# zkonduit/ezkl

Measured on AMD Instinct MI355X. Metric: BN254 G1 MSM pts/s (2^20 points per GPU; NTT 2^22 elems/s in extra), higher is better.
Workload: dtype u32x8 (254-bit modular integer, Montgomery); 1 GPU; configs[1]: standalone 2^20-point BN254 G1 MSM (uniform scalars, try-and-increment bases) + 2^22 scalar-field NTT per GPU; parallelism=points sharded across 1 rank(s); all_gather of 64-B partials + host fold

## Files before the change

### ezkl_amd/backend.py

```python
import ctypes as C
import numpy as np
from . import lib as _l

_vp = C.c_void_p


def _p(a):
    return a.ctypes.data_as(_vp)


def _fe(a, shape_last=4):
    a = np.ascontiguousarray(a, dtype=np.uint64)
    if a.shape[-1] != shape_last:
        raise ValueError("expected trailing dimension %d" % shape_last)
    return a


def init(device=-1):
    _l.check(_l.load().ezkl_hip_init(C.c_int(device)), "ezkl_hip_init")


def synchronize():
    _l.check(_l.load().ezkl_hip_synchronize(), "ezkl_hip_synchronize")

# ... 293 lines not shown
    num_poly = message.shape[0] // n + 1
    polys = np.zeros((num_poly, n_rows, 4), np.uint64)
    polys[:, n:, :] = _to_mont(1)
    for i in range(message.shape[0]):
        polys[i // n, i % n] = message[i]
    out = np.zeros((num_poly, 8), np.uint64)
    arr = (C.c_void_p * num_poly)(*[polys[j].ctypes.data for j in range(num_poly)])
    _l.check(_l.load().ezkl_hip_msm_g1_batch(params._gl.h, arr, C.c_size_t(num_poly), C.c_size_t(n_rows), _p(out)),
             "ezkl_hip_msm_g1_batch")
    return out


def msm_g2(points, scalars):
    points, scalars = _fe(points, 16), _fe(scalars)
    if points.shape[0] != scalars.shape[0]:
        raise ValueError("one scalar per point")
    out = np.zeros(16, np.uint64)
    _l.check(_l.load().ezkl_hip_msm_g2(_p(points), _p(scalars), C.c_size_t(points.shape[0]), _p(out)), "ezkl_hip_msm_g2")
    return out


def g1_add_affine(a, b):
    a, b = _fe(a, 8), _fe(b, 8)
    out = np.zeros(8, np.uint64)
    _l.check(_l.load().ezkl_hip_g1_add_affine(_p(a), _p(b), _p(out)), "ezkl_hip_g1_add_affine")
    return out


def ntt(a, log_n, omega, inverse=False):
    a = _fe(a).copy()
    w = _fe(omega)
    _l.check(_l.load().ezkl_hip_ntt(_p(a), C.c_uint32(log_n), _p(w), C.c_int(1 if inverse else 0)), "ezkl_hip_ntt")
    return a


def ntt_dev(ptr, log_n, omega, inverse=False, batch=1, stride=None, stream=None):
    w = _fe(omega)
    stride = (1 << log_n) if stride is None else stride
    _l.check(_l.load().ezkl_hip_ntt_dev(_vp(ptr), C.c_uint32(log_n), _p(w), C.c_int(1 if inverse else 0),
                                         C.c_size_t(batch), C.c_size_t(stride), _stream_ptr(stream)), "ezkl_hip_ntt_dev")


def set_async(on):
    prev = C.c_int(0)
    _l.check(_l.load().ezkl_hip_set_async(C.c_int(1 if on else 0), C.byref(prev)), "ezkl_hip_set_async")
    return bool(prev.value)


def vec_op(op, a_ptr, b_ptr, out_ptr, n, stream=None):
    code = {"add": 0, "sub": 1, "mul": 2}[op]
    _l.check(_l.load().ezkl_hip_vec_op_dev(C.c_int(code), _vp(a_ptr), _vp(b_ptr), _vp(out_ptr), C.c_size_t(n),
                                            _stream_ptr(stream)), "ezkl_hip_vec_op_dev")


def permutation_sigma_dev(next_ptr, omega_col_ptr, delta_pows_ptr, n_columns, log_n, out_ptr, stream=None):
    _l.check(_l.load().ezkl_hip_permutation_sigma_dev(_vp(next_ptr), _vp(omega_col_ptr), _vp(delta_pows_ptr), C.c_uint32(n_columns), C.c_uint32(log_n),
                                                      _vp(out_ptr), _stream_ptr(stream)), "ezkl_hip_permutation_sigma_dev")


def vec_scale(a_ptr, scalar, out_ptr, n, stream=None):
    _l.check(_l.load().ezkl_hip_vec_scale_dev(_vp(a_ptr), _p(_fe(scalar)), _vp(out_ptr), C.c_size_t(n), _stream_ptr(stream)), "ezkl_hip_vec_scale_dev")


def vec_fill(out_ptr, value, n, stream=None):
    _l.check(_l.load().ezkl_hip_vec_fill_dev(_vp(out_ptr), _p(_fe(value)), C.c_size_t(n), _stream_ptr(stream)), "ezkl_hip_vec_fill_dev")


def coset_ntt_dev(in_ptr, out_ptr, k, ext_k, inverse=False, in_len=None, batch=1, stream=None):
    nin = (1 << ext_k) if inverse else (1 << k)
    _l.check(_l.load().ezkl_hip_coset_ntt_dev(_vp(in_ptr), _vp(out_ptr), C.c_size_t(batch), C.c_size_t(nin), C.c_size_t(1 << ext_k),
                                               C.c_uint32(k), C.c_uint32(ext_k), C.c_int(1 if inverse else 0), _stream_ptr(stream)),
             "ezkl_hip_coset_ntt_dev")


def coeff_to_cosets_dev(in_ptr, out_ptr, k, ext_k, batch=1, stream=None):
    _l.check(_l.load().ezkl_hip_coeff_to_cosets_dev(_vp(in_ptr), _vp(out_ptr), C.c_size_t(batch), C.c_size_t(1 << k), C.c_size_t(1 << ext_k),
                                                     C.c_uint32(k), C.c_uint32(ext_k), _stream_ptr(stream)), "ezkl_hip_coeff_to_cosets_dev")


def coeff_to_cosets_range_dev(in_ptr, out_ptr, k, ext_k, first_coset, n_cosets, batch=1, stream=None):
    _l.check(_l.load().ezkl_hip_coeff_to_cosets_range_dev(_vp(in_ptr), _vp(out_ptr), C.c_size_t(batch), C.c_size_t(1 << k), C.c_size_t(n_cosets << k),
                                                           C.c_uint32(k), C.c_uint32(ext_k), C.c_uint32(first_coset), C.c_uint32(n_cosets), _stream_ptr(stream)),
             "ezkl_hip_coeff_to_cosets_range_dev")


def cosets_transpose_dev(in_ptr, out_ptr, k, ext_k, to_natural=True, stream=None):
    _l.check(_l.load().ezkl_hip_cosets_transpose_dev(_vp(in_ptr), _vp(out_ptr), C.c_uint32(k), C.c_uint32(ext_k), C.c_int(1 if to_natural else 0),
                                                      _stream_ptr(stream)), "ezkl_hip_cosets_transpose_dev")


def divide_by_vanishing_dev(ptr, k, ext_k, stream=None):
    _l.check(_l.load().ezkl_hip_divide_by_vanishing_dev(_vp(ptr), C.c_uint32(k), C.c_uint32(ext_k), _stream_ptr(stream)),
             "ezkl_hip_divide_by_vanishing_dev")


def memcpy_h2d(dst_ptr, arr):
    arr = np.ascontiguousarray(arr)
    _l.check(_l.load().ezkl_hip_memcpy_h2d(_vp(dst_ptr), _p(arr), C.c_size_t(arr.nbytes)), "h2d")


def memcpy_d2h(src_ptr, nbytes):
    out = np.empty(nbytes, np.uint8)
    _l.check(_l.load().ezkl_hip_memcpy_d2h(_p(out), _vp(src_ptr), C.c_size_t(nbytes)), "d2h")
    return out


def prefix_scan(op, in_ptr, out_ptr, n, exclusive=False, stream=None):
    code = {"add": 0, "mul": 2}[op]
    _l.check(_l.load().ezkl_hip_prefix_scan_dev(C.c_int(code), C.c_int(1 if exclusive else 0), _vp(in_ptr), _vp(out_ptr),
                                                 C.c_size_t(n), _stream_ptr(stream)), "ezkl_hip_prefix_scan_dev")


def lookup_multiplicity(input_ptrs, table_ptr, n_rows, usable_rows, stream=None):
    out = DeviceBuffer(n_rows * 32)
    miss = C.c_uint32(0)
    arr = (C.c_void_p * max(1, len(input_ptrs)))(*input_ptrs)
    _l.check(_l.load().ezkl_hip_lookup_multiplicity_dev(arr, C.c_uint32(len(input_ptrs)), _vp(table_ptr), C.c_uint32(n_rows),
                                                         C.c_uint32(usable_rows), _vp(out.ptr), C.byref(miss), _stream_ptr(stream)),
             "ezkl_hip_lookup_multiplicity_dev")
    return out, int(miss.value)


def lookup_multiplicity_batch(inputs_per_lookup, table_ptrs, n_rows, usable_rows, stream=None):
    L = len(table_ptrs)
    outs = [DeviceBuffer(n_rows * 32) for _ in range(L)]
    flat = [p for ins in inputs_per_lookup for p in ins]
    which = [l for l, ins in enumerate(inputs_per_lookup) for _ in ins]
    miss = DeviceBuffer.from_numpy(np.zeros(1, np.uint32))
    a_in = (C.c_void_p * max(1, len(flat)))(*flat)
    a_which = (C.c_uint32 * max(1, len(which)))(*which)
    a_tab = (C.c_void_p * L)(*table_ptrs)
    a_out = (C.c_void_p * L)(*[o.ptr for o in outs])
    _l.check(_l.load().ezkl_hip_lookup_multiplicity_batch_dev(a_in, a_which, C.c_uint32(len(flat)), a_tab, C.c_uint32(L), C.c_uint32(n_rows), C.c_uint32(usable_rows),
                                                               a_out, _vp(miss.ptr), _stream_ptr(stream)), "ezkl_hip_lookup_multiplicity_batch_dev")
    return outs, int(miss.to_numpy(np.uint32, (1,))[0])


def _records(rec, counters, cap):
    cnt = counters.to_numpy(np.uint64)
    m = int(min(cnt[0], cap))
    r = rec.to_numpy(np.uint32)[:4 * m].reshape(m, 4) if m else np.zeros((0, 4), np.uint32)
    return [tuple(int(x) for x in row) for row in r], [int(x) for x in cnt]


def lookup_missing_rows(inputs_per_lookup, table_ptrs, n_rows, usable_rows, cap=1024, stream=None):
    L = len(table_ptrs)
    flat = [p for ins in inputs_per_lookup for p in ins]
    which = [l for l, ins in enumerate(inputs_per_lookup) for _ in ins]
    rec, cnt = DeviceBuffer(max(1, cap) * 16), DeviceBuffer.from_numpy(np.zeros(1 + L, np.uint64))
    a_in = (C.c_void_p * max(1, len(flat)))(*flat)
    a_which = (C.c_uint32 * max(1, len(which)))(*which)
    a_tab = (C.c_void_p * L)(*table_ptrs)
    _l.check(_l.load().ezkl_hip_lookup_missing_rows_dev(a_in, a_which, C.c_uint32(len(flat)), a_tab, C.c_uint32(L), C.c_uint32(n_rows), C.c_uint32(usable_rows),
                                                         _vp(rec.ptr), C.c_uint32(cap), _vp(cnt.ptr), _stream_ptr(stream)), "ezkl_hip_lookup_missing_rows_dev")
    return _records(rec, cnt, cap)


def copy_check(col_ptrs, next_ptr, log_n, cap=1024, stream=None):
    rec, cnt = DeviceBuffer(max(1, cap) * 16), DeviceBuffer.from_numpy(np.zeros(1, np.uint64))
    a = (C.c_void_p * max(1, len(col_ptrs)))(*col_ptrs)
    _l.check(_l.load().ezkl_hip_copy_check_dev(a, C.c_uint32(len(col_ptrs)), _vp(next_ptr), C.c_uint32(log_n), _vp(rec.ptr), C.c_uint32(cap), _vp(cnt.ptr),
                                                _stream_ptr(stream)), "ezkl_hip_copy_check_dev")
    return _records(rec, cnt, cap)


def eval_polynomial(coeffs_ptr, n, x, stream=None):
# ... 516 lines not shown
```

### ezkl_amd/csrc/capi.hip

```cpp
#include "common.hpp"
#include <string.h>
#include <atomic>
#include <algorithm>
#include <iterator>

namespace ezkl {

static std::mutex g_init_mu;
static constexpr int MAX_CTX = 64;
static std::atomic<Ctx*> g_ctxs[MAX_CTX];
static int g_ctx_device[MAX_CTX];
static std::atomic<int> g_n_ctx{0};
static thread_local int t_ctx = 0;
static std::atomic<int> g_last_hip_err{0};

int set_hip_error(hipError_t e, const char* what, const char* file, int line) {
    g_last_hip_err.store((int)e);
    fprintf(stderr, "[ezkl_hip] HIP error %d (%s) at %s:%d in %s\n", (int)e, hipGetErrorString(e), file, line, what);
    (void)hipGetLastError();
    return e == hipErrorOutOfMemory ? EZKL_ERR_NOMEM : EZKL_ERR_HIP;
}

static int device_count_checked(int* n) {
    *n = 0;
// ... 768 lines not shown
    for (size_t i = 0; i < count; i++)
        if (!scalars_dev[i]) return EZKL_ERR_INVALID;
    EZ_CTX(c);
    return msm_batch_push_many(c, reinterpret_cast<MsmBatch*>(batch), (const fe_t* const*)scalars_dev, count, c->stream);
}
int ezkl_hip_msm_batch_finish(ezkl_msm_batch_t batch, void* out, size_t capacity) {
    if (!batch || (!out && capacity)) return EZKL_ERR_INVALID;
    EZ_CTX(c);
    return msm_batch_finish(c, reinterpret_cast<MsmBatch*>(batch), out, capacity);
}
int ezkl_hip_g1_add_affine(const void* a, const void* b, void* out) {
    if (!a || !b || !out) return EZKL_ERR_INVALID;
    g1_add_affine_host(a, b, out);
    return EZKL_OK;
}

int ezkl_hip_ntt_dev(void* data, uint32_t log_n, const void* omega, int inverse, size_t batch, size_t stride, void* stream) {
    if (!data || !omega || batch == 0) return EZKL_ERR_INVALID;
    EZ_CTX(c);
    fe_t w;
    memcpy(&w, omega, 32);
    hipStream_t st = pick_stream(c, stream);
    int rc = ntt_run(c, st, (const fe_t*)data, (fe_t*)data, log_n, w, inverse != 0, batch, stride, stride, log_n, 0);
    if (rc) return rc;
    return finish(c, st, stream);
}
int ezkl_hip_ntt(void* data, uint32_t log_n, const void* omega, int inverse) {
    if (!data || !omega || log_n > 28) return EZKL_ERR_INVALID;
    EZ_CTX(c);
    size_t bytes = (size_t)32 << log_n;
    fe_t* d = nullptr;
    EZ_HIP(hipMalloc(&d, bytes));
    int rc = EZKL_OK;
    hipError_t e = hipMemcpyAsync(d, data, bytes, hipMemcpyHostToDevice, c->stream);
    if (e != hipSuccess) rc = set_hip_error(e, "h2d", __FILE__, __LINE__);
    if (!rc) rc = ezkl_hip_ntt_dev(d, log_n, omega, inverse, 1, (size_t)1 << log_n, nullptr);
    if (!rc) {
        e = copy_sync(c, data, d, bytes, hipMemcpyDeviceToHost);
        if (e != hipSuccess) rc = set_hip_error(e, "d2h", __FILE__, __LINE__);
    }
    (void)hipFree(d);
    return rc;
}

static fe_t domain_omega(uint32_t k, bool inverse) {
    fe_t w = fr_const(FrConst::ROOT);
    for (uint32_t i = k; i < 28; i++) w = Fr::sqr(w);
    return inverse ? Fr::inv(w) : w;
}

int ezkl_hip_coset_ntt_dev(const void* in, void* out, size_t batch, size_t in_stride, size_t out_stride,
                           uint32_t log_n, uint32_t log_n_ext, int inverse, void* stream) {
    if (!in || !out || batch == 0 || log_n > log_n_ext || log_n_ext > 28) return EZKL_ERR_INVALID;
    EZ_CTX(c);
    hipStream_t st = pick_stream(c, stream);
    fe_t w = domain_omega(log_n_ext, inverse != 0);
    int rc;
    if (!inverse)
        rc = ntt_run(c, st, (const fe_t*)in, (fe_t*)out, log_n_ext, w, false, batch, in_stride, out_stride, log_n, 1);
    else
        rc = ntt_run(c, st, (const fe_t*)in, (fe_t*)out, log_n_ext, w, true, batch, in_stride, out_stride, log_n_ext, 2);
    if (rc) return rc;
    return finish(c, st, stream);
}
int ezkl_hip_coeff_to_cosets_dev(const void* in, void* out, size_t batch, size_t in_stride, size_t out_stride, uint32_t log_n, uint32_t log_n_ext, void* stream) {
    if (!in || !out || in == out || batch == 0 || log_n > log_n_ext || log_n_ext > 28 || log_n_ext - log_n > 6) return EZKL_ERR_INVALID;
    EZ_CTX(c);
    hipStream_t st = pick_stream(c, stream);
    int rc = coset_cm_run(c, st, (const fe_t*)in, (fe_t*)out, log_n, log_n_ext, domain_omega(log_n, false), domain_omega(log_n_ext, false), batch, in_stride, out_stride);
    if (rc) return rc;
    return finish(c, st, stream);
}
int ezkl_hip_coeff_to_cosets_range_dev(const void* in, void* out, size_t batch, size_t in_stride, size_t out_stride, uint32_t log_n, uint32_t log_n_ext,
                                       uint32_t first_coset, uint32_t n_cosets, void* stream) {
    if (!in || !out || in == out || batch == 0 || log_n > log_n_ext || log_n_ext > 28 || log_n_ext - log_n > 6) return EZKL_ERR_INVALID;
    if (n_cosets == 0 || (n_cosets & (n_cosets - 1)) || (uint64_t)first_coset + n_cosets > (1ull << (log_n_ext - log_n))) return EZKL_ERR_INVALID;
    EZ_CTX(c);
    hipStream_t st = pick_stream(c, stream);
    int rc = coset_cm_run(c, st, (const fe_t*)in, (fe_t*)out, log_n, log_n_ext, domain_omega(log_n, false), domain_omega(log_n_ext, false), batch, in_stride, out_stride,
                          first_coset, n_cosets);
    if (rc) return rc;
    return finish(c, st, stream);
}
int ezkl_hip_cosets_transpose_dev(const void* in, void* out, uint32_t log_n, uint32_t log_n_ext, int to_natural, void* stream) {
    if (!in || !out || in == out || log_n > log_n_ext || log_n_ext > 28) return EZKL_ERR_INVALID;
    EZ_CTX(c);
    hipStream_t st = pick_stream(c, stream);
    int rc = cm_transpose(c, st, (const fe_t*)in, (fe_t*)out, log_n, log_n_ext - log_n, to_natural != 0);
    if (rc) return rc;
    return finish(c, st, stream);
}
int ezkl_hip_coset_ntt_batch(const void* const* in, void* const* out, size_t batch, uint32_t log_n, uint32_t log_n_ext, int inverse) {
    if (!in || !out || log_n > log_n_ext || log_n_ext > 28) return EZKL_ERR_INVALID;
    EZ_CTX(c);
    const size_t ne = (size_t)1 << log_n_ext, nin = inverse ? ne : ((size_t)1 << log_n);
    fe_t *din = nullptr, *dout = nullptr;
    EZ_HIP(hipMalloc(&din, nin * 32));
    EZ_HIP(hipMalloc(&dout, ne * 32));
    int rc = EZKL_OK;
    for (size_t b = 0; b < batch && !rc; b++) {
        hipError_t e = hipMemcpyAsync(din, in[b], nin * 32, hipMemcpyHostToDevice, c->stream);
        if (e != hipSuccess) { rc = set_hip_error(e, "h2d", __FILE__, __LINE__); break; }
        rc = ezkl_hip_coset_ntt_dev(din, dout, 1, nin, ne, log_n, log_n_ext, inverse, nullptr);
        if (rc) break;
        e = copy_sync(c, out[b], dout, ne * 32, hipMemcpyDeviceToHost);
        if (e != hipSuccess) rc = set_hip_error(e, "d2h", __FILE__, __LINE__);
    }
    (void)hipFree(din);
    (void)hipFree(dout);
    return rc;
}

int ezkl_hip_vec_op_dev(int op, const void* a, const void* b, void* o, size_t n, void* stream) {
    if (!a || !b || !o || op < 0 || op > 2) return EZKL_ERR_INVALID;
    EZ_CTX(c);
    hipStream_t st = pick_stream(c, stream);
    int rc = vec_op(c, st, op, (const fe_t*)a, (const fe_t*)b, (fe_t*)o, n);
    return rc ? rc : finish(c, st, stream);
}
int ezkl_hip_vec_fill_dev(void* o, const void* v, size_t n, void* stream) {
    if (!o || !v) return EZKL_ERR_INVALID;
    EZ_CTX(c);
    fe_t val;
    memcpy(&val, v, 32);
    hipStream_t st = pick_stream(c, stream);
    int rc = vec_fill(c, st, (fe_t*)o, val, n);
    return rc ? rc : finish(c, st, stream);
}
int ezkl_hip_permutation_sigma_dev(const void* next_dev, const void* omega_col_dev, const void* delta_pows_dev, uint32_t n_columns, uint32_t log_n,
                                   void* out_dev, void* stream) {
    if (!next_dev || !omega_col_dev || !delta_pows_dev || !out_dev || n_columns == 0 || log_n > 28) return EZKL_ERR_INVALID;
    if (((uint64_t)n_columns << log_n) > ((uint64_t)1 << 32)) return EZKL_ERR_INVALID;
    EZ_CTX(c);
    hipStream_t st = pick_stream(c, stream);
    int rc = perm_sigma(c, st, (const uint32_t*)next_dev, (const fe_t*)omega_col_dev, (const fe_t*)delta_pows_dev, log_n, n_columns, (fe_t*)out_dev);
    return rc ? rc : finish(c, st, stream);
}
int ezkl_hip_vec_scale_dev(const void* a, const void* s, void* o, size_t n, void* stream) {
    if (!a || !s || !o) return EZKL_ERR_INVALID;
    EZ_CTX(c);
    fe_t sc;
    memcpy(&sc, s, 32);
    hipStream_t st = pick_stream(c, stream);
    int rc = vec_scale(c, st, (const fe_t*)a, sc, (fe_t*)o, n);
    return rc ? rc : finish(c, st, stream);
}
int ezkl_hip_divide_by_vanishing_dev(void* a, uint32_t k, uint32_t ext_k, void* stream) {
    if (!a || k > ext_k || ext_k > 28) return EZKL_ERR_INVALID;
    EZ_CTX(c);
    return divide_by_vanishing(c, pick_stream(c, stream), (fe_t*)a, k, ext_k);
}
int ezkl_hip_batch_invert_dev(void* a, size_t n, void* stream) {
    if (!a) return EZKL_ERR_INVALID;
    EZ_CTX(c);
    hipStream_t st = pick_stream(c, stream);
    int rc = batch_invert(c, st, (fe_t*)a, n);
    return rc ? rc : finish(c, st, stream);
}

int ezkl_hip_lookup_multiplicity_dev(const void* const* inputs_dev, uint32_t n_inputs, const void* table_dev, uint32_t n_rows,
                                     uint32_t usable_rows, void* m_out_dev, uint32_t* out_missing, void* stream) {
    if (!table_dev || !m_out_dev || (n_inputs && !inputs_dev)) return EZKL_ERR_INVALID;
    for (uint32_t j = 0; j < n_inputs; j++)
        if (!inputs_dev[j]) return EZKL_ERR_INVALID;
    EZ_CTX(c);
    return lookup_multiplicity(c, pick_stream(c, stream), (const fe_t* const*)inputs_dev, n_inputs, (const fe_t*)table_dev, n_rows,
// ... 178 lines not shown
```

### ezkl_amd/csrc/common.hpp

```cpp
#pragma once
#include <hip/hip_runtime.h>
#include <stdint.h>
#include <stdio.h>
#include <map>
#include <mutex>
#include <string>
#include <vector>
#include <rocprofiler-sdk-roctx/roctx.h>
#include "../../include/ezkl_hip.h"
#include "field.hpp"

namespace ezkl {

struct Ctx {
    int device = -1;
    hipStream_t stream = nullptr;
    hipEvent_t order_event = nullptr;
    int num_cus = 256;
    std::recursive_mutex mu;
    struct EvRing {
        static constexpr unsigned N = 64;
        hipEvent_t e0[N], e1[N];
        bool made[N];
        uint64_t head = 0, tail = 0;
        double sum_ms = 0;
        uint64_t count = 0, skipped = 0;
        EvRing() { for (unsigned i = 0; i < N; i++) { e0[i] = e1[i] = nullptr; made[i] = false; } }
    };
    std::map<std::string, EvRing> events;
    struct Arena {
        void* ptr = nullptr;
        size_t bytes = 0;
        hipStream_t last_stream = nullptr;
        hipEvent_t last_event = nullptr;
        bool in_use = false;
    };
    Arena scratch, aux;
    std::map<hipStream_t, Arena> scratch_by_stream;
    void* msm_state = nullptr;
    void* ntt_state = nullptr;
    void* jit_state = nullptr;
    void* pool_state = nullptr;
    int index = 0;
    void* staging_state = nullptr;
    hipStream_t side_stream = nullptr;
};

Ctx* ctx();
int ctx_init(int device);
int ctx_count();
int ctx_bind(int idx);
int ctx_device_of(int idx);
int set_hip_error(hipError_t e, const char* what, const char* file, int line);
int arena_reserve(Ctx::Arena& a, size_t bytes, hipStream_t st, void** out);
int arena_done(Ctx::Arena& a, hipStream_t st);
int ev_pair(Ctx* c, const char* key, hipEvent_t* e0, hipEvent_t* e1);
int ev_harvest(Ctx::EvRing& r, bool all);
uint8_t* staging_acquire(Ctx* c, size_t bytes, void** token);
int staging_release(void* token, hipStream_t st);

#define EZ_HIP(call)                                                              \
    do {                                                                          \
        hipError_t _e = (call);                                                   \
        if (_e != hipSuccess) return ::ezkl::set_hip_error(_e, #call, __FILE__, __LINE__); \
    } while (0)

struct RoctxRange {
    explicit RoctxRange(const char* name) { roctxRangePushA(name); }
    ~RoctxRange() { roctxRangePop(); }
};

#define EZ_CTX(c)                                   \
    ::ezkl::RoctxRange _roctx(__func__);            \
    ::ezkl::Ctx* c = ::ezkl::ctx();                 \
    if (!c) return EZKL_ERR_NO_DEVICE;              \
    std::lock_guard<std::recursive_mutex> _lk(c->mu); \
    EZ_HIP(hipSetDevice(c->device))

static inline hipError_t stream_create_prio(hipStream_t* st, const char* env_name, int dflt) {
    int prio = dflt;
    if (const char* e = getenv(env_name)) prio = atoi(e);
    int lo = 0, hi = 0;
    if (hipDeviceGetStreamPriorityRange(&lo, &hi) != hipSuccess) { (void)hipGetLastError(); return hipStreamCreateWithFlags(st, hipStreamNonBlocking); }
    if (prio > lo) prio = lo;
    if (prio < hi) prio = hi;
    if (prio == 0) return hipStreamCreateWithFlags(st, hipStreamNonBlocking);
    return hipStreamCreateWithPriority(st, hipStreamNonBlocking, prio);
}
static inline Ctx::Arena& scratch_arena(Ctx* c, hipStream_t st) { return st == c->stream ? c->scratch : c->scratch_by_stream[st]; }
static inline hipStream_t pick_stream(Ctx* c, void* s) { return s ? (hipStream_t)s : c->stream; }
static inline unsigned cdiv(size_t a, size_t b) { return (unsigned)((a + b - 1) / b); }

struct Bases {
    fe_t* pts = nullptr;
    size_t n = 0;
};

int ntt_run(Ctx* c, hipStream_t st, const fe_t* in, fe_t* out, uint32_t log_n, const fe_t& omega, bool inverse_scale,
            size_t batch, size_t in_stride, size_t out_stride, uint32_t in_log_len, int coset_mode);
int coset_cm_run(Ctx* c, hipStream_t st, const fe_t* in, fe_t* out, uint32_t log_n, uint32_t log_ext, const fe_t& w_n, const fe_t& w_ext, size_t batch,
                 size_t in_stride, size_t out_stride, uint32_t first_coset = 0, uint32_t n_cosets = 0);
int cm_transpose(Ctx* c, hipStream_t st, const fe_t* in, fe_t* out, uint32_t log_n, uint32_t log_e, bool to_natural);
int msm_run(Ctx* c, hipStream_t st, const Bases* b, size_t base_offset, const fe_t* scalars_dev, size_t n,
            void* out_affine_host);
int msm_run_batch(Ctx* c, hipStream_t st, const Bases* b, size_t base_offset, const fe_t* const* scalars, size_t batch, size_t n,
                  void* out_host, bool small_scalars = false);
struct MsmUpload;
int msm_upload_begin(Ctx* c, const fe_t* const* host_cols, fe_t* const* dev_cols, size_t batch, size_t n, const fe_t* const* tails, size_t tail_start,
                     size_t tail_count, MsmUpload** out, const uint8_t* formats = nullptr);
int msm_upload_wait(MsmUpload* u, size_t j, hipStream_t st);
int msm_upload_commit(Ctx* c, MsmUpload* u, const Bases* b, size_t commit_first, size_t commit_count, void* out_host);
int msm_upload_end(MsmUpload* u);
struct MsmBatch;
int msm_batch_begin(Ctx* c, hipStream_t st, const Bases* b, size_t base_offset, size_t n, MsmBatch** out);
int msm_batch_push(Ctx* c, MsmBatch* mb, const fe_t* scalars_dev);
int msm_batch_push_many(Ctx* c, MsmBatch* mb, const fe_t* const* cols, size_t count, hipStream_t after);
int msm_batch_finish(Ctx* c, MsmBatch* mb, void* out_host, size_t capacity);
int vec_op(Ctx* c, hipStream_t st, int op, const fe_t* a, const fe_t* b, fe_t* o, size_t n);
int vec_fill(Ctx* c, hipStream_t st, fe_t* o, const fe_t& v, size_t n);
int vec_scale(Ctx* c, hipStream_t st, const fe_t* a, const fe_t& s, fe_t* o, size_t n);
int perm_sigma(Ctx* c, hipStream_t st, const uint32_t* next, const fe_t* omega_col, const fe_t* delta_pows, uint32_t log_n, uint32_t m, fe_t* out);
int divide_by_vanishing(Ctx* c, hipStream_t st, fe_t* a, uint32_t k, uint32_t ext_k);
int batch_invert(Ctx* c, hipStream_t st, fe_t* a, size_t n);
int lookup_multiplicity_batch(Ctx* c, hipStream_t st, const fe_t* const* inputs, const uint32_t* which, uint32_t n_items, const fe_t* const* tables,
                              uint32_t n_lookups, uint32_t n_rows, uint32_t usable, fe_t* const* m_outs, uint32_t* missing_host, uint32_t* missing_dev);
int lookup_multiplicity(Ctx* c, hipStream_t st, const fe_t* const* inputs, uint32_t n_inputs, const fe_t* table, uint32_t n_rows,
                        uint32_t usable, fe_t* m_out, uint32_t* missing_host, uint32_t* missing_dev);
int eval_poly(Ctx* c, hipStream_t st, const fe_t* coeffs, size_t n, const fe_t& x, void* out_host);
int prefix_scan(Ctx* c, hipStream_t st, int op, int exclusive, const fe_t* in, fe_t* out, size_t n);
int eval_poly_batch(Ctx* c, hipStream_t st, const fe_t* const* coeffs, const fe_t* xs, uint32_t m, size_t n, void* out_host);
int lincomb(Ctx* c, hipStream_t st, const fe_t* const* in, const fe_t* coeffs, uint32_t m, fe_t* out, size_t n, int accumulate);
int kate_division(Ctx* c, hipStream_t st, const fe_t* a, const fe_t& z, fe_t* out, size_t n);
int chacha20_fr(Ctx* c, hipStream_t st, const uint32_t key[8], uint64_t stream, size_t first, fe_t* out, size_t n);
bool msm_upload_is_open();
int msm_run_concurrent(Ctx* c, std::unique_lock<std::recursive_mutex>& lk, const Bases* b, size_t base_offset, const fe_t* scalars, size_t n, void* out_host);
int msm_call_start(Ctx* c, std::unique_lock<std::recursive_mutex>& lk, const Bases* b, size_t base_offset, const fe_t* scalars, size_t n, int* slot_out);
int msm_call_finish(Ctx* c, std::unique_lock<std::recursive_mutex>& lk, int slot, void* out_host);
int eval_program(Ctx* c, hipStream_t st, const ezkl_program_t* p, fe_t* out, bool ordered);
int eval_jit_compile_only(const ezkl_program_t* p);
int eval_jit_source_only(const ezkl_program_t* p, char* out, size_t cap, size_t* len);
int eval_check_source_only(const ezkl_program_t* p, const uint32_t* slots, uint32_t n_checks, char* out, size_t cap, size_t* len);
int eval_check(Ctx* c, hipStream_t st, const ezkl_program_t* p, const uint32_t* slots, uint32_t n_checks, uint32_t row_lo, uint32_t row_hi, void* rec,
               uint32_t cap, void* count);
int lookup_missing_rows(Ctx* c, hipStream_t st, const fe_t* const* inputs, const uint32_t* which, uint32_t n_items, const fe_t* const* tables,
                        uint32_t n_lookups, uint32_t n_rows, uint32_t usable, void* rec, uint32_t cap, void* count);
int copy_check(Ctx* c, hipStream_t st, const fe_t* const* cols, uint32_t m, const uint32_t* next, uint32_t log_n, void* rec, uint32_t cap, void* count);
int eval_prepare(Ctx* c, const ezkl_program_t* p);
int eval_schedule_only(const ezkl_program_t* p, uint32_t* out_code);
void eval_jit_stats(uint64_t* compiled, uint64_t* from_disk, uint64_t* hits);
int ubench(Ctx* c, const char* which, double* out);
void msm_table_drop(const Bases* b);
int msm_table_prepare(Ctx* c, const Bases* b);
int g1_mul_fixed(Ctx* c, hipStream_t st, const void* base_host, const fe_t* scalars, size_t n, void* out_dev);
int gen_bases(Ctx* c, hipStream_t st, uint64_t seed, size_t first, size_t n, void* out_dev);
int g1_to_lagrange(Ctx* c, hipStream_t st, const void* g_dev, uint32_t log_n, fe_t* tw_mont, const fe_t& ninv_mont, void* out_dev);
void g1_add_affine_host(const void* a, const void* b, void* out);
int g2_msm(Ctx* c, hipStream_t st, const void* pts_host, const void* scalars_host, size_t n, void* out_host);

}
```

### ezkl_amd/csrc/field29.hpp

```cpp
#pragma once
#include "field.hpp"
#include "montmul29_gen.hpp"

#ifndef EZKL_FQ29_ILP
#define EZKL_FQ29_ILP 0
#endif
#ifndef EZKL_FUSED_Y
#define EZKL_FUSED_Y 1
#endif
namespace ezkl {

struct f29_t {
    uint32_t v[9];
};
static constexpr uint32_t M29 = (1u << 29) - 1;

template <class CT, bool IS_FQ>
struct Field29 {
    typedef CT C;
    typedef uint32_t u32x9 __attribute__((ext_vector_type(9)));
    EZ_D static void mul_asm(const uint32_t (&a)[9], const uint32_t (&b)[9], uint32_t (&r)[9]) {
        if (IS_FQ) {
#if EZKL_FQ29_ILP
            mont_mul29i_fq(a, b, r);
#else
            mont_mul29_fq(a, b, r);
#endif
        } else mont_mul29_fr(a, b, r);
    }

    EZ_D static f29_t zero() {
        f29_t r;
#pragma unroll
        for (int i = 0; i < 9; i++) r.v[i] = 0;
        return r;
    }
    EZ_D static f29_t one() {
        f29_t r;
#pragma unroll
        for (int i = 0; i < 9; i++) r.v[i] = C::ONE[i];
        return r;
    }
    EZ_D static bool limbs_zero(const f29_t& a) {
        uint32_t o = 0;
#pragma unroll
        for (int i = 0; i < 9; i++) o |= a.v[i];
        return o == 0;
    }
    __device__ __attribute__((noinline)) static u32x9 mul_call(u32x9 a, u32x9 b) {
        uint32_t x[9], y[9], r[9];
#pragma unroll
        for (int i = 0; i < 9; i++) { x[i] = a[i]; y[i] = b[i]; }
        mul_asm(x, y, r);
        u32x9 o;
#pragma unroll
        for (int i = 0; i < 9; i++) o[i] = r[i];
        return o;
    }
    EZ_D static f29_t mul(const f29_t& a, const f29_t& b) {
        f29_t r;
        mul_asm(a.v, b.v, r.v);
        return r;
    }
    EZ_D static f29_t mul2add(const f29_t& a, const f29_t& b, const f29_t& c, const f29_t& d) {
        static_assert(IS_FQ, "generated for Fq only");
        f29_t r;
        mont_mul2add29_fq(a.v, b.v, c.v, d.v, r.v);
        return r;
    }
    EZ_D static f29_t mul_cold(const f29_t& a, const f29_t& b) {
        u32x9 x, y;
#pragma unroll
        for (int i = 0; i < 9; i++) { x[i] = a.v[i]; y[i] = b.v[i]; }
        u32x9 o = mul_call(x, y);
        f29_t r;
#pragma unroll
        for (int i = 0; i < 9; i++) r.v[i] = o[i];
        return r;
    }
    EZ_D static f29_t sqr(const f29_t& a) {
        f29_t r;
        if (IS_FQ) {
#if EZKL_FQ29_ILP
            mont_sqr29i_fq(a.v, r.v);
#else
            mont_sqr29_fq(a.v, r.v);
#endif
        } else mont_sqr29_fr(a.v, r.v);
        return r;
    }
    EZ_D static f29_t sqr_cold(const f29_t& a) { return mul_cold(a, a); }
    EZ_D static f29_t add(const f29_t& a, const f29_t& b) {
        f29_t r;
#pragma unroll
        for (int i = 0; i < 9; i++) r.v[i] = a.v[i] + b.v[i];
        return r;
    }
    template <int KI>
    EZ_D static f29_t sub(const f29_t& a, const f29_t& b) {
        f29_t r;
#pragma unroll
        for (int i = 0; i < 9; i++) r.v[i] = a.v[i] + (C::SUBC[KI][i] - b.v[i]);
        return r;
    }
    template <int KI>
    EZ_D static f29_t neg(const f29_t& b) {
        f29_t r;
#pragma unroll
        for (int i = 0; i < 9; i++) r.v[i] = C::SUBC[KI][i] - b.v[i];
        return r;
    }
    EZ_D static f29_t normalize(const f29_t& a) {
        f29_t r = a;
#pragma unroll
        for (int i = 0; i < 8; i++) {
            r.v[i + 1] += r.v[i] >> 29;
            r.v[i] &= M29;
        }
        return r;
    }
    EZ_D static bool is_zero_mod_p(const f29_t& a) {
        const uint32_t j = (a.v[0] * C::P0INV) & M29;
        if (j >= 32) return false;
        uint32_t carry = 0, diff = 0;
#pragma unroll
        for (int i = 0; i < 9; i++) {
            const uint64_t t = (uint64_t)j * C::P[i] + carry;
            const uint32_t limb = i < 8 ? ((uint32_t)t & M29) : (uint32_t)t;
            carry = i < 8 ? (uint32_t)(t >> 29) : 0;
            diff |= limb ^ a.v[i];
        }
        return diff == 0;
    }
    template <int KI>
    EZ_D static f29_t cond_sub(const f29_t& x) {
        f29_t t;
#pragma unroll
        for (int i = 0; i < 9; i++) t.v[i] = x.v[i] + C::CSUB[KI][i];
        t = normalize(t);
        const bool ge = (t.v[8] >> 29) != 0;
        t.v[8] &= M29;
        f29_t r;
#pragma unroll
        for (int i = 0; i < 9; i++) r.v[i] = ge ? t.v[i] : x.v[i];
        return r;
    }
    EZ_D static f29_t canonical(const f29_t& x) {
        constexpr uint32_t D = (uint32_t)(C::P[8] + 1u);
        constexpr uint64_t MAGIC = (((uint64_t)1 << 51) + D - 1) / D;
        const uint32_t q = (uint32_t)(((uint64_t)x.v[8] * MAGIC) >> 51);
        f29_t r;
        uint64_t acc = 0;
#pragma unroll
        for (int i = 0; i < 9; i++) {
            acc += (uint64_t)q * C::CSUB[0][i] + x.v[i];
            r.v[i] = (uint32_t)acc & M29;
            acc >>= 29;
        }
        return cond_sub<0>(r);
    }
    EZ_D static fe_t pack(const f29_t& a) {
        fe_t w;
#pragma unroll
        for (int j = 0; j < 8; j++) {
            const int bit = 32 * j, lo = bit / 29, sh = bit - 29 * lo;
            uint32_t acc = a.v[lo] >> sh;
            const int have = 29 - sh;
            if (lo + 1 < 9) acc |= a.v[lo + 1] << have;
            if (have + 29 < 32 && lo + 2 < 9) acc |= a.v[lo + 2] << (have + 29);
            w.v[j] = acc;
        }
        return w;
    }
    EZ_D static f29_t unpack(const fe_t& w) {
        f29_t r;
#pragma unroll
        for (int i = 0; i < 8; i++) {
            const int bit = 29 * i, word = bit >> 5, sh = bit & 31;
            const uint32_t lo = w.v[word], hi = word + 1 < 8 ? w.v[word + 1] : 0u;
            r.v[i] = (sh ? __builtin_amdgcn_alignbit(hi, lo, sh) : lo) & M29;
        }
        r.v[8] = w.v[7] >> 8;
        return r;
    }
};

typedef Field29<Fq29C, true> Fq29;
typedef Field29<Fr29C, false> Fr29;

EZ_D f29_t ld_f29(const f29_t* p) {
    f29_t r;
#pragma unroll
    for (int i = 0; i < 9; i++) r.v[i] = p->v[i];
    return r;
}
EZ_D void st_f29(f29_t* p, const f29_t& a) {
#pragma unroll
    for (int i = 0; i < 9; i++) p->v[i] = a.v[i];
}

}
```

### ezkl_amd/csrc/montmul29_gen.hpp

```cpp
#pragma once
#ifndef __HIPCC_RTC__
#include <stdint.h>
#endif
namespace ezkl {
struct Fq29C {
    static constexpr uint32_t P[9] = {0x187cfd47u, 0x010460b6u, 0x1c72a34fu, 0x02d522d0u, 0x1585d978u, 0x02db40c0u, 0x00a6e141u, 0x0e5c2634u, 0x0030644eu};
    static constexpr uint32_t ONE[9] = {0x157ccc21u, 0x141c2758u, 0x185230d3u, 0x014c0419u, 0x0aa36fb9u, 0x1d4240ceu, 0x11d54c07u, 0x052ac7a8u, 0x000dc836u};
    static constexpr uint32_t P0INV = 0x1b799c77u;
    static constexpr uint32_t SUBC[7][9] = {
        {0x30f9fa8eu, 0x2208c16cu, 0x38e5469du, 0x25aa45a0u, 0x2b0bb2efu, 0x25b68180u, 0x214dc281u, 0x3cb84c67u, 0x0060c89bu},
        {0x21f3f51cu, 0x241182dau, 0x31ca8d3bu, 0x2b548b42u, 0x361765dfu, 0x2b6d0301u, 0x229b8503u, 0x397098cfu, 0x00c19138u},
        {0x23e7ea38u, 0x282305b5u, 0x23951a77u, 0x36a91686u, 0x2c2ecbbfu, 0x36da0604u, 0x25370a07u, 0x32e1319fu, 0x01832272u},
        {0x27cfd470u, 0x30460b6bu, 0x272a34efu, 0x2d522d0du, 0x385d9780u, 0x2db40c09u, 0x2a6e1410u, 0x25c2633fu, 0x030644e6u},
        {0x2f9fa8e0u, 0x208c16d7u, 0x2e5469e0u, 0x3aa45a1bu, 0x30bb2f01u, 0x3b681814u, 0x34dc2821u, 0x2b84c67fu, 0x060c89cdu},
        {0x3f3f51c0u, 0x21182dafu, 0x3ca8d3c1u, 0x3548b437u, 0x21765e04u, 0x36d0302au, 0x29b85044u, 0x37098d00u, 0x0c19139bu},
        {0x3e7ea380u, 0x22305b60u, 0x3951a783u, 0x2a916870u, 0x22ecbc0au, 0x2da06055u, 0x3370a08au, 0x2e131a01u, 0x18322738u},
    };
    static constexpr uint32_t CSUB[4][9] = {
        {0x078302b9u, 0x1efb9f49u, 0x038d5cb0u, 0x1d2add2fu, 0x0a7a2687u, 0x1d24bf3fu, 0x1f591ebeu, 0x11a3d9cbu, 0x1fcf9bb1u},
        {0x0f060572u, 0x1df73e92u, 0x071ab961u, 0x1a55ba5eu, 0x14f44d0fu, 0x1a497e7eu, 0x1eb23d7du, 0x0347b397u, 0x1f9f3763u},
        {0x1e0c0ae4u, 0x1bee7d24u, 0x0e3572c3u, 0x14ab74bcu, 0x09e89a1fu, 0x1492fcfdu, 0x1d647afbu, 0x068f672fu, 0x1f3e6ec6u},
        {0x1c1815c8u, 0x17dcfa49u, 0x1c6ae587u, 0x0956e978u, 0x13d1343fu, 0x0925f9fau, 0x1ac8f5f7u, 0x0d1ece5fu, 0x1e7cdd8cu},
    };
    static constexpr uint32_t R261_32[8] = {0x157ccc21u, 0x4e8384ebu, 0x0ce148c3u, 0xfb90a602u, 0x819caa36u, 0x5301fa84u, 0x563d4475u, 0x0dc83629u};
};
struct Fr29C {
    static constexpr uint32_t P[9] = {0x10000001u, 0x1f0fac9fu, 0x0e5c2450u, 0x07d090f3u, 0x1585d283u, 0x02db40c0u, 0x00a6e141u, 0x0e5c2634u, 0x0030644eu};
    static constexpr uint32_t ONE[9] = {0x0fffff57u, 0x1ea70ab4u, 0x052c068bu, 0x17504f49u, 0x0aa8075bu, 0x1d4240ceu, 0x11d54c07u, 0x052ac7a8u, 0x000dc836u};
    static constexpr uint32_t P0INV = 0x10000001u;
    static constexpr uint32_t SUBC[7][9] = {
        {0x20000002u, 0x3e1f593eu, 0x3cb848a0u, 0x2fa121e5u, 0x2b0ba505u, 0x25b68180u, 0x214dc281u, 0x3cb84c67u, 0x0060c89bu},
        {0x20000004u, 0x3c3eb27du, 0x39709142u, 0x3f4243ccu, 0x36174a0bu, 0x2b6d0301u, 0x229b8503u, 0x397098cfu, 0x00c19138u},
        {0x20000008u, 0x387d64fbu, 0x32e12286u, 0x3e84879au, 0x2c2e9418u, 0x36da0604u, 0x25370a07u, 0x32e1319fu, 0x01832272u},
        {0x20000010u, 0x30fac9f7u, 0x25c2450eu, 0x3d090f36u, 0x385d2832u, 0x2db40c09u, 0x2a6e1410u, 0x25c2633fu, 0x030644e6u},
        {0x20000020u, 0x21f593efu, 0x2b848a1eu, 0x3a121e6du, 0x30ba5066u, 0x3b681814u, 0x34dc2821u, 0x2b84c67fu, 0x060c89cdu},
        {0x20000040u, 0x23eb27dfu, 0x3709143du, 0x34243cdbu, 0x2174a0ceu, 0x36d0302au, 0x29b85044u, 0x37098d00u, 0x0c19139bu},
        {0x20000080u, 0x27d64fbfu, 0x2e12287bu, 0x284879b8u, 0x22e9419eu, 0x2da06055u, 0x3370a08au, 0x2e131a01u, 0x18322738u},
    };
    static constexpr uint32_t CSUB[4][9] = {
        {0x0fffffffu, 0x00f05360u, 0x11a3dbafu, 0x182f6f0cu, 0x0a7a2d7cu, 0x1d24bf3fu, 0x1f591ebeu, 0x11a3d9cbu, 0x1fcf9bb1u},
        {0x1ffffffeu, 0x01e0a6c0u, 0x0347b75eu, 0x105ede19u, 0x14f45af9u, 0x1a497e7eu, 0x1eb23d7du, 0x0347b397u, 0x1f9f3763u},
        {0x1ffffffcu, 0x03c14d81u, 0x068f6ebcu, 0x00bdbc32u, 0x09e8b5f3u, 0x1492fcfdu, 0x1d647afbu, 0x068f672fu, 0x1f3e6ec6u},
        {0x1ffffff8u, 0x07829b03u, 0x0d1edd78u, 0x017b7864u, 0x13d16be6u, 0x0925f9fau, 0x1ac8f5f7u, 0x0d1ece5fu, 0x1e7cdd8cu},
    };
    static constexpr uint32_t R261_32[8] = {0x8fffff57u, 0x2fd4e156u, 0xa494b01au, 0x75bba827u, 0x819caa80u, 0x5301fa84u, 0x563d4475u, 0x0dc83629u};
};
__device__ __forceinline__ void mont_mul29_fq(const uint32_t (&a)[9], const uint32_t (&b)[9], uint32_t (&r)[9]) {
    asm("s_mov_b32 s16, 0x187cfd47\n\t"
        "s_mov_b32 s17, 0x010460b6\n\t"
        "s_mov_b32 s18, 0x1c72a34f\n\t"
        "s_mov_b32 s19, 0x02d522d0\n\t"
        "s_mov_b32 s20, 0x1585d978\n\t"
        "s_mov_b32 s21, 0x02db40c0\n\t"
        "s_mov_b32 s22, 0x00a6e141\n\t"
        "s_mov_b32 s23, 0x0e5c2634\n\t"
        "s_mov_b32 s24, 0x0030644e\n\t"
        "s_mov_b32 s25, 0x04866389\n\t"
        "s_mov_b32 s26, 0x1fffffff\n\t"
        "v_mad_u64_u32 v[16:17], vcc, %[a0], %[b0], 0\n\t"
        "v_mul_lo_u32 %[r0], v16, s25\n\t"
        "v_and_b32 %[r0], s26, %[r0]\n\t"
        "v_mad_u64_u32 v[16:17], vcc, %[r0], s16, v[16:17]\n\t"
        "v_lshrrev_b64 v[16:17], 29, v[16:17]\n\t"
        "v_mad_u64_u32 v[16:17], vcc, %[a0], %[b1], v[16:17]\n\t"
        "v_mad_u64_u32 v[16:17], vcc, %[a1], %[b0], v[16:17]\n\t"
        "v_mad_u64_u32 v[16:17], vcc, %[r0], s17, v[16:17]\n\t"
        "v_mul_lo_u32 %[r1], v16, s25\n\t"
        "v_and_b32 %[r1], s26, %[r1]\n\t"
        "v_mad_u64_u32 v[16:17], vcc, %[r1], s16, v[16:17]\n\t"
        "v_lshrrev_b64 v[16:17], 29, v[16:17]\n\t"
        "v_mad_u64_u32 v[16:17], vcc, %[a0], %[b2], v[16:17]\n\t"
        "v_mad_u64_u32 v[16:17], vcc, %[a1], %[b1], v[16:17]\n\t"
        "v_mad_u64_u32 v[16:17], vcc, %[a2], %[b0], v[16:17]\n\t"
        "v_mad_u64_u32 v[16:17], vcc, %[r0], s18, v[16:17]\n\t"
        "v_mad_u64_u32 v[16:17], vcc, %[r1], s17, v[16:17]\n\t"
        "v_mul_lo_u32 %[r2], v16, s25\n\t"
        "v_and_b32 %[r2], s26, %[r2]\n\t"
        "v_mad_u64_u32 v[16:17], vcc, %[r2], s16, v[16:17]\n\t"
        "v_lshrrev_b64 v[16:17], 29, v[16:17]\n\t"
        "v_mad_u64_u32 v[16:17], vcc, %[a0], %[b3], v[16:17]\n\t"
        "v_mad_u64_u32 v[16:17], vcc, %[a1], %[b2], v[16:17]\n\t"
        "v_mad_u64_u32 v[16:17], vcc, %[a2], %[b1], v[16:17]\n\t"
        "v_mad_u64_u32 v[16:17], vcc, %[a3], %[b0], v[16:17]\n\t"
        "v_mad_u64_u32 v[16:17], vcc, %[r0], s19, v[16:17]\n\t"
        "v_mad_u64_u32 v[16:17], vcc, %[r1], s18, v[16:17]\n\t"
        "v_mad_u64_u32 v[16:17], vcc, %[r2], s17, v[16:17]\n\t"
        "v_mul_lo_u32 %[r3], v16, s25\n\t"
        "v_and_b32 %[r3], s26, %[r3]\n\t"
        "v_mad_u64_u32 v[16:17], vcc, %[r3], s16, v[16:17]\n\t"
        "v_lshrrev_b64 v[16:17], 29, v[16:17]\n\t"
        "v_mad_u64_u32 v[16:17], vcc, %[a0], %[b4], v[16:17]\n\t"
        "v_mad_u64_u32 v[16:17], vcc, %[a1], %[b3], v[16:17]\n\t"
        "v_mad_u64_u32 v[16:17], vcc, %[a2], %[b2], v[16:17]\n\t"
        "v_mad_u64_u32 v[16:17], vcc, %[a3], %[b1], v[16:17]\n\t"
        "v_mad_u64_u32 v[16:17], vcc, %[a4], %[b0], v[16:17]\n\t"
        "v_mad_u64_u32 v[16:17], vcc, %[r0], s20, v[16:17]\n\t"
        "v_mad_u64_u32 v[16:17], vcc, %[r1], s19, v[16:17]\n\t"
        "v_mad_u64_u32 v[16:17], vcc, %[r2], s18, v[16:17]\n\t"
        "v_mad_u64_u32 v[16:17], vcc, %[r3], s17, v[16:17]\n\t"
        "v_mul_lo_u32 %[r4], v16, s25\n\t"
        "v_and_b32 %[r4], s26, %[r4]\n\t"
        "v_mad_u64_u32 v[16:17], vcc, %[r4], s16, v[16:17]\n\t"
        "v_lshrrev_b64 v[16:17], 29, v[16:17]\n\t"
        "v_mad_u64_u32 v[16:17], vcc, %[a0], %[b5], v[16:17]\n\t"
        "v_mad_u64_u32 v[16:17], vcc, %[a1], %[b4], v[16:17]\n\t"
        "v_mad_u64_u32 v[16:17], vcc, %[a2], %[b3], v[16:17]\n\t"
        "v_mad_u64_u32 v[16:17], vcc, %[a3], %[b2], v[16:17]\n\t"
        "v_mad_u64_u32 v[16:17], vcc, %[a4], %[b1], v[16:17]\n\t"
        "v_mad_u64_u32 v[16:17], vcc, %[a5], %[b0], v[16:17]\n\t"
        "v_mad_u64_u32 v[16:17], vcc, %[r0], s21, v[16:17]\n\t"
        "v_mad_u64_u32 v[16:17], vcc, %[r1], s20, v[16:17]\n\t"
        "v_mad_u64_u32 v[16:17], vcc, %[r2], s19, v[16:17]\n\t"
        "v_mad_u64_u32 v[16:17], vcc, %[r3], s18, v[16:17]\n\t"
        "v_mad_u64_u32 v[16:17], vcc, %[r4], s17, v[16:17]\n\t"
        "v_mul_lo_u32 %[r5], v16, s25\n\t"
        "v_and_b32 %[r5], s26, %[r5]\n\t"
        "v_mad_u64_u32 v[16:17], vcc, %[r5], s16, v[16:17]\n\t"
        "v_lshrrev_b64 v[16:17], 29, v[16:17]\n\t"
        "v_mad_u64_u32 v[16:17], vcc, %[a0], %[b6], v[16:17]\n\t"
        "v_mad_u64_u32 v[16:17], vcc, %[a1], %[b5], v[16:17]\n\t"
        "v_mad_u64_u32 v[16:17], vcc, %[a2], %[b4], v[16:17]\n\t"
        "v_mad_u64_u32 v[16:17], vcc, %[a3], %[b3], v[16:17]\n\t"
        "v_mad_u64_u32 v[16:17], vcc, %[a4], %[b2], v[16:17]\n\t"
        "v_mad_u64_u32 v[16:17], vcc, %[a5], %[b1], v[16:17]\n\t"
        "v_mad_u64_u32 v[16:17], vcc, %[a6], %[b0], v[16:17]\n\t"
        "v_mad_u64_u32 v[16:17], vcc, %[r0], s22, v[16:17]\n\t"
        "v_mad_u64_u32 v[16:17], vcc, %[r1], s21, v[16:17]\n\t"
        "v_mad_u64_u32 v[16:17], vcc, %[r2], s20, v[16:17]\n\t"
// ... 1665 lines not shown
        "v_mad_u64_u32 v[16:17], vcc, %[r5], s20, v[16:17]\n\t"
        "v_mad_u64_u32 v[18:19], vcc, %[a7], %[b3], v[18:19]\n\t"
        "v_mad_u64_u32 v[16:17], vcc, %[r6], s19, v[16:17]\n\t"
        "v_mad_u64_u32 v[18:19], vcc, %[a8], %[b2], v[18:19]\n\t"
        "v_mad_u64_u32 v[16:17], vcc, %[r7], s18, v[16:17]\n\t"
        "v_mad_u64_u32 v[16:17], vcc, %[r8], s17, v[16:17]\n\t"
        "v_and_b32 %[r0], s26, v16\n\t"
        "v_lshrrev_b64 v[16:17], 29, v[16:17]\n\t"
        "v_lshl_add_u64 v[16:17], v[18:19], 0, v[16:17]\n\t"
        "v_mad_u64_u32 v[18:19], vcc, %[a3], %[b8], 0\n\t"
        "v_mad_u64_u32 v[16:17], vcc, %[r2], s24, v[16:17]\n\t"
        "v_mad_u64_u32 v[18:19], vcc, %[a4], %[b7], v[18:19]\n\t"
        "v_mad_u64_u32 v[16:17], vcc, %[r3], s23, v[16:17]\n\t"
        "v_mad_u64_u32 v[18:19], vcc, %[a5], %[b6], v[18:19]\n\t"
        "v_mad_u64_u32 v[16:17], vcc, %[r4], s22, v[16:17]\n\t"
        "v_mad_u64_u32 v[18:19], vcc, %[a6], %[b5], v[18:19]\n\t"
        "v_mad_u64_u32 v[16:17], vcc, %[r5], s21, v[16:17]\n\t"
        "v_mad_u64_u32 v[18:19], vcc, %[a7], %[b4], v[18:19]\n\t"
        "v_mad_u64_u32 v[16:17], vcc, %[r6], s20, v[16:17]\n\t"
        "v_mad_u64_u32 v[18:19], vcc, %[a8], %[b3], v[18:19]\n\t"
        "v_mad_u64_u32 v[16:17], vcc, %[r7], s19, v[16:17]\n\t"
        "v_mad_u64_u32 v[16:17], vcc, %[r8], s18, v[16:17]\n\t"
        "v_and_b32 %[r1], s26, v16\n\t"
        "v_lshrrev_b64 v[16:17], 29, v[16:17]\n\t"
        "v_lshl_add_u64 v[16:17], v[18:19], 0, v[16:17]\n\t"
        "v_mad_u64_u32 v[18:19], vcc, %[a4], %[b8], 0\n\t"
        "v_mad_u64_u32 v[16:17], vcc, %[r3], s24, v[16:17]\n\t"
        "v_mad_u64_u32 v[18:19], vcc, %[a5], %[b7], v[18:19]\n\t"
        "v_mad_u64_u32 v[16:17], vcc, %[r4], s23, v[16:17]\n\t"
        "v_mad_u64_u32 v[18:19], vcc, %[a6], %[b6], v[18:19]\n\t"
        "v_mad_u64_u32 v[16:17], vcc, %[r5], s22, v[16:17]\n\t"
        "v_mad_u64_u32 v[18:19], vcc, %[a7], %[b5], v[18:19]\n\t"
        "v_mad_u64_u32 v[16:17], vcc, %[r6], s21, v[16:17]\n\t"
        "v_mad_u64_u32 v[18:19], vcc, %[a8], %[b4], v[18:19]\n\t"
        "v_mad_u64_u32 v[16:17], vcc, %[r7], s20, v[16:17]\n\t"
        "v_mad_u64_u32 v[16:17], vcc, %[r8], s19, v[16:17]\n\t"
        "v_and_b32 %[r2], s26, v16\n\t"
        "v_lshrrev_b64 v[16:17], 29, v[16:17]\n\t"
        "v_lshl_add_u64 v[16:17], v[18:19], 0, v[16:17]\n\t"
        "v_mad_u64_u32 v[18:19], vcc, %[a5], %[b8], 0\n\t"
        "v_mad_u64_u32 v[16:17], vcc, %[r4], s24, v[16:17]\n\t"
        "v_mad_u64_u32 v[18:19], vcc, %[a6], %[b7], v[18:19]\n\t"
        "v_mad_u64_u32 v[16:17], vcc, %[r5], s23, v[16:17]\n\t"
        "v_mad_u64_u32 v[18:19], vcc, %[a7], %[b6], v[18:19]\n\t"
        "v_mad_u64_u32 v[16:17], vcc, %[r6], s22, v[16:17]\n\t"
        "v_mad_u64_u32 v[18:19], vcc, %[a8], %[b5], v[18:19]\n\t"
        "v_mad_u64_u32 v[16:17], vcc, %[r7], s21, v[16:17]\n\t"
        "v_mad_u64_u32 v[16:17], vcc, %[r8], s20, v[16:17]\n\t"
        "v_and_b32 %[r3], s26, v16\n\t"
        "v_lshrrev_b64 v[16:17], 29, v[16:17]\n\t"
        "v_lshl_add_u64 v[16:17], v[18:19], 0, v[16:17]\n\t"
        "v_mad_u64_u32 v[18:19], vcc, %[a6], %[b8], 0\n\t"
        "v_mad_u64_u32 v[16:17], vcc, %[r5], s24, v[16:17]\n\t"
        "v_mad_u64_u32 v[18:19], vcc, %[a7], %[b7], v[18:19]\n\t"
        "v_mad_u64_u32 v[16:17], vcc, %[r6], s23, v[16:17]\n\t"
        "v_mad_u64_u32 v[18:19], vcc, %[a8], %[b6], v[18:19]\n\t"
        "v_mad_u64_u32 v[16:17], vcc, %[r7], s22, v[16:17]\n\t"
        "v_mad_u64_u32 v[16:17], vcc, %[r8], s21, v[16:17]\n\t"
        "v_and_b32 %[r4], s26, v16\n\t"
        "v_lshrrev_b64 v[16:17], 29, v[16:17]\n\t"
        "v_lshl_add_u64 v[16:17], v[18:19], 0, v[16:17]\n\t"
        "v_mad_u64_u32 v[18:19], vcc, %[a7], %[b8], 0\n\t"
        "v_mad_u64_u32 v[16:17], vcc, %[r6], s24, v[16:17]\n\t"
        "v_mad_u64_u32 v[18:19], vcc, %[a8], %[b7], v[18:19]\n\t"
        "v_mad_u64_u32 v[16:17], vcc, %[r7], s23, v[16:17]\n\t"
        "v_mad_u64_u32 v[16:17], vcc, %[r8], s22, v[16:17]\n\t"
        "v_and_b32 %[r5], s26, v16\n\t"
        "v_lshrrev_b64 v[16:17], 29, v[16:17]\n\t"
        "v_lshl_add_u64 v[16:17], v[18:19], 0, v[16:17]\n\t"
        "v_mad_u64_u32 v[18:19], vcc, %[a8], %[b8], 0\n\t"
        "v_mad_u64_u32 v[16:17], vcc, %[r7], s24, v[16:17]\n\t"
        "v_mad_u64_u32 v[16:17], vcc, %[r8], s23, v[16:17]\n\t"
        "v_and_b32 %[r6], s26, v16\n\t"
        "v_lshrrev_b64 v[16:17], 29, v[16:17]\n\t"
        "v_lshl_add_u64 v[16:17], v[18:19], 0, v[16:17]\n\t"
        "v_mad_u64_u32 v[16:17], vcc, %[r8], s24, v[16:17]\n\t"
        "v_and_b32 %[r7], s26, v16\n\t"
        "v_lshrrev_b64 v[16:17], 29, v[16:17]\n\t"
        "v_mov_b32 %[r8], v16\n\t"
        : [r0] "=&v"(r[0]), [r1] "=&v"(r[1]), [r2] "=&v"(r[2]), [r3] "=&v"(r[3]), [r4] "=&v"(r[4]), [r5] "=&v"(r[5]), [r6] "=&v"(r[6]), [r7] "=&v"(r[7]), [r8] "=&v"(r[8])
        : [a0] "v"(a[0]), [a1] "v"(a[1]), [a2] "v"(a[2]), [a3] "v"(a[3]), [a4] "v"(a[4]), [a5] "v"(a[5]), [a6] "v"(a[6]), [a7] "v"(a[7]), [a8] "v"(a[8]), [b0] "v"(b[0]), [b1] "v"(b[1]), [b2] "v"(b[2]), [b3] "v"(b[3]), [b4] "v"(b[4]), [b5] "v"(b[5]), [b6] "v"(b[6]), [b7] "v"(b[7]), [b8] "v"(b[8])
        : "v16", "v17", "v18", "v19", "s16", "s17", "s18", "s19", "s20", "s21", "s22", "s23", "s24", "s25", "s26", "vcc");
}
}
```

### ezkl_amd/csrc/ntt.hip

```cpp
#include "common.hpp"
#include "field29.hpp"
#include <string.h>


namespace ezkl {

static constexpr uint32_t NTT_LOG_TILE = 10;
static constexpr uint32_t NTT_LOG_SINGLE = 11;

struct PassArgs {
    const fe_t* in;
    fe_t* out;
    size_t in_stride, out_stride;
    const fe_t* tw_inter;
    uint32_t log_n, log_r, log_m, log_tile;
    uint32_t last, first;
    uint32_t in_log_len;
    uint32_t coset_pre;
    uint32_t post;
    uint32_t npass, log_radix[4];
    uint32_t k1_major;
    fe_t zeta[2];
    fe_t post_c[3];
    uint32_t cm, cm_log_e, cm_first, cm_log_cnt;
    const f29_t* tw_stage29;
    const f29_t* tw_pre29;
    uint32_t lds_stages;
};

EZ_D void lds_put29(uint2* d, uint32_t* d8, uint32_t tile, uint32_t e, const f29_t& x) {
#pragma unroll
    for (int q = 0; q < 4; q++) d[q * tile + e] = make_uint2(x.v[2 * q], x.v[2 * q + 1]);
    d8[e] = x.v[8];
}
EZ_D f29_t lds_get29(const uint2* d, const uint32_t* d8, uint32_t tile, uint32_t e) {
    f29_t x;
#pragma unroll
    for (int q = 0; q < 4; q++) {
        uint2 t = d[q * tile + e];
        x.v[2 * q] = t.x;
        x.v[2 * q + 1] = t.y;
    }
    x.v[8] = d8[e];
    return x;
}
template <int G, int NTT_THREADS, bool FROM_TABLE>
__device__ __forceinline__ void ntt_superstage29(uint2* data, uint32_t* d8, const f29_t* tw, uint32_t TILE, uint32_t logC, bool unit1, uint32_t s, uint32_t tid) {
    constexpr uint32_t M = 1u << G;
    const uint32_t C = 1u << logC;
    const uint32_t lh = s - 1, h = 1u << lh;
    const uint32_t ngroups = TILE >> G;
    for (uint32_t gid = tid; gid < ngroups; gid += NTT_THREADS) {
        const uint32_t c = gid & (C - 1), q = gid >> logC;
        const uint32_t o = q & (h - 1), blk = q >> lh;
        const uint32_t r0 = (blk << (lh + G)) + o;
        f29_t x[M];
#pragma unroll
        for (uint32_t i = 0; i < M; i++) x[i] = lds_get29(data, d8, TILE, ((r0 + i * h) << logC) + c);
#pragma unroll
        for (int t = 0; t < G; t++) {
            const uint32_t half = 1u << t, st = s + t;
            const uint32_t base = (1u << (st - 1)) - 1u;
#pragma unroll
            for (uint32_t i = 0; i < M; i++) {
                if (i & half) continue;
                if (unit1 && st == 1) {
                    const f29_t v = x[i + half];
                    x[i + half] = Fr29::sub<2>(x[i], v);
                    x[i] = Fr29::add(x[i], v);
                } else if (unit1 && st == 2 && (i & 1u) == 0) {
                    const f29_t v = Fr29::normalize(x[i + half]);
                    x[i + half] = Fr29::sub<4>(x[i], v);
                    x[i] = Fr29::add(x[i], v);
                } else {
                    const uint32_t off = o + (i & (half - 1)) * h;
                    const f29_t w = ld_f29(tw + base + off);
                    const f29_t v = Fr29::mul(x[i + half], w);
                    x[i + half] = Fr29::sub<1>(x[i], v);
                    x[i] = Fr29::add(x[i], v);
                }
            }
        }
#pragma unroll
        for (uint32_t i = 0; i < M; i++) lds_put29(data, d8, TILE, ((r0 + i * h) << logC) + c, Fr29::normalize(x[i]));
    }
}

template <int NTT_THREADS>
__global__ __launch_bounds__(NTT_THREADS) void ntt_pass_kernel(PassArgs a) {
    extern __shared__ __attribute__((aligned(16))) unsigned char smem[];
    const uint32_t TILE = 1u << a.log_tile;
    const uint32_t logC = a.log_tile - a.log_r, C = 1u << logC;
    const uint32_t log_s = a.log_m - a.log_r, S = 1u << log_s;
    uint2* data = reinterpret_cast<uint2*>(smem);
    uint32_t* d8 = reinterpret_cast<uint32_t*>(smem + 32u * TILE);
    f29_t* tloc = reinterpret_cast<f29_t*>(smem + 36u * TILE);
    const uint32_t tid = threadIdx.x, tile = blockIdx.x;
    const uint32_t cm_l = a.cm ? (blockIdx.y & ((1u << a.cm_log_cnt) - 1u)) : 0u, cm_col = a.cm ? (blockIdx.y >> a.cm_log_cnt) : blockIdx.y;
    const uint32_t cm_b = a.cm_first + cm_l;
    const bool twisted = a.cm && a.first;
    const fe_t* in = a.in + (size_t)(twisted ? cm_col : blockIdx.y) * a.in_stride;
    fe_t* out = (a.cm && a.last) ? a.out + (size_t)cm_col * a.out_stride + ((size_t)cm_l << a.log_n) : a.out + (size_t)blockIdx.y * a.out_stride;
    const fe_t* tw_inter = a.tw_inter ? a.tw_inter + (twisted ? ((size_t)cm_b << a.log_n) : 0) : nullptr;
    const f29_t* tws = twisted ? a.tw_pre29 + ((size_t)cm_b << a.log_r) : a.tw_stage29;
    for (uint32_t j = tid; j + 1 < (1u << a.lds_stages); j += NTT_THREADS) st_f29(tloc + j, ld_f29(tws + j));

    uint32_t n_blocks = 1u << (a.log_n - a.log_r);
    uint32_t sblk = a.npass >= 2 ? (n_blocks >> a.log_radix[0]) : 1u;
    auto col_base = [&](uint32_t c) -> size_t {
        if (!a.last) {
            uint32_t colid = tile * C + c;
            return ((size_t)(colid >> log_s) << a.log_m) + (colid & (S - 1));
        }
        uint32_t blk;
        if (a.k1_major) {
            uint32_t rest = tile % sblk, k10 = (tile / sblk) * C;
            blk = (k10 + c) * sblk + rest;
        } else {
            blk = tile * C + c;
        }
        return (size_t)blk << a.log_r;
    };

    const size_t in_len = (size_t)1 << a.in_log_len;
    auto load_one = [&](uint32_t e, size_t& addr_out) -> fe_t {
        uint32_t c = e & (C - 1), i1 = e >> logC;
        size_t addr = col_base(c) + ((size_t)i1 << log_s);
        addr_out = addr;
        if (!a.first || addr < in_len) return ld_fe(in + addr);
        return Fr::zero();
    };
    auto put_one = [&](uint32_t e, size_t addr, const fe_t& raw) {
        f29_t x = Fr29::unpack(raw);
        if (a.first && a.coset_pre && addr < in_len) {
            uint32_t m3 = (uint32_t)(addr % 3);
            if (m3) x = Fr29::mul(x, Fr29::unpack(a.zeta[m3 - 1]));
        }
        e = (a.log_r ? ((__brev(e >> logC) >> (32 - a.log_r)) << logC) : 0u) | (e & (C - 1));
        lds_put29(data, d8, TILE, e, x);
    };
    if (TILE == 4 * NTT_THREADS) {
        fe_t x[4];
        size_t ad[4];
#pragma unroll
        for (int i = 0; i < 4; i++) x[i] = load_one(tid + i * NTT_THREADS, ad[i]);
#pragma unroll
        for (int i = 0; i < 4; i++) put_one(tid + i * NTT_THREADS, ad[i], x[i]);
    } else {
        for (uint32_t e = tid; e < TILE; e += NTT_THREADS) {
            size_t ad;
            fe_t x = load_one(e, ad);
            put_one(e, ad, x);
        }
    }
    __syncthreads();

    for (uint32_t s = 1; s <= a.log_r;) {
        const uint32_t g = a.log_r - s >= 1 ? 2u : 1u;
        if (s > a.lds_stages) {
            if (g == 2) ntt_superstage29<2, NTT_THREADS, true>(data, d8, tws, TILE, logC, !twisted, s, tid);
            else ntt_superstage29<1, NTT_THREADS, true>(data, d8, tws, TILE, logC, !twisted, s, tid);
        } else {
            if (g == 2) ntt_superstage29<2, NTT_THREADS, false>(data, d8, tloc, TILE, logC, !twisted, s, tid);
            else ntt_superstage29<1, NTT_THREADS, false>(data, d8, tloc, TILE, logC, !twisted, s, tid);
        }
        __syncthreads();
        s += g;
    }

    auto store_one = [&](uint32_t e, const fe_t* twp) {
        uint32_t c = e & (C - 1), k1 = e >> logC;
        f29_t x = lds_get29(data, d8, TILE, (k1 << logC) + c);
        if (!a.last) {
            uint32_t colid = tile * C + c;
            uint32_t pos = (k1 << log_s) + (colid & (S - 1));
            x = Fr29::mul(x, Fr29::unpack(twp ? *twp : ld_fe(tw_inter + pos)));
            st_fe(out + (((size_t)(colid >> log_s) << a.log_m) + pos), Fr29::pack(x));
        } else {
            uint32_t blk = (uint32_t)(col_base(c) >> a.log_r);
            size_t oidx = 0;
            uint32_t rem = blk, lw = a.log_n - a.log_r, shift = 0;
            for (uint32_t p = 0; p + 1 < a.npass; p++) {
                lw -= a.log_radix[p];
                uint32_t kp = rem >> lw;
                rem &= (1u << lw) - 1;
                oidx += (size_t)kp << shift;
                shift += a.log_radix[p];
            }
            oidx += (size_t)k1 << shift;
            x = a.post ? Fr29::cond_sub<0>(Fr29::mul(x, Fr29::unpack(a.post_c[oidx % 3]))) : Fr29::canonical(x);
            st_fe(out + oidx, Fr29::pack(x));
        }
    };
    if (TILE == 4 * NTT_THREADS && !a.last) {
        fe_t tw[4];
#pragma unroll
        for (int i = 0; i < 4; i++) {
            uint32_t e = tid + i * NTT_THREADS, c = e & (C - 1), k1 = e >> logC;
            tw[i] = ld_fe(tw_inter + ((k1 << log_s) + ((tile * C + c) & (S - 1))));
        }
#pragma unroll
        for (int i = 0; i < 4; i++) store_one(tid + i * NTT_THREADS, &tw[i]);
    } else {
        for (uint32_t e = tid; e < TILE; e += NTT_THREADS) store_one(e, nullptr);
    }
}

__global__ void ntt_twiddle_kernel(fe_t* out, uint32_t count, uint64_t mult, uint32_t log_n, uint32_t log_s,
                                   int mode, const fe_t* pow2tab, fe_t init) {
    uint32_t idx = blockIdx.x * blockDim.x + threadIdx.x;
    if (idx >= count) return;
    uint64_t e;
    if (mode == 0) e = (uint64_t)idx * mult;
    else e = (uint64_t)(idx & ((1u << log_s) - 1)) * (uint64_t)(idx >> log_s) * mult;
    e &= ((uint64_t)1 << log_n) - 1;
    fe_t acc = init;
    for (uint32_t b = 0; b < log_n; b++)
        if ((e >> b) & 1) acc = Fr::mul(acc, ld_fe(pow2tab + b));
    st_fe(out + idx, acc);
}


__global__ void ntt_coset_table_kernel(fe_t* out, f29_t* out29, uint32_t cnt, uint32_t log_e, uint32_t log_ext, uint32_t log_s, int mode, const fe_t* pow2tab,
                                       fe_t z0, fe_t z1, fe_t z2) {
    const size_t idx = (size_t)blockIdx.x * blockDim.x + threadIdx.x;
    if (idx >= ((size_t)cnt << log_e)) return;
    const uint64_t b = idx / cnt, m = idx % cnt;
    uint64_t e, z;
    if (mode == 0) {
        uint32_t st = 1;
        while (((uint64_t)1 << st) - 1 <= m) st++;
        const uint64_t o = m - (((uint64_t)1 << (st - 1)) - 1), log_nn = log_ext - log_e;
        if (st > log_nn) {
            if (out29) st_f29(out29 + idx, Fr29::zero());
            else st_fe(out + idx, Fr::zero());
            return;
        }
        const uint64_t q = (uint64_t)1 << (log_nn - st);
        e = q * (b + (o << log_e));
        z = q % 3;
    } else {
        const uint64_t i2 = m & (((uint64_t)1 << log_s) - 1), k1 = m >> log_s;
        e = ((i2 * k1) << log_e) + b * i2;
        z = i2 % 3;
    }
    e &= ((uint64_t)1 << log_ext) - 1;
    fe_t acc = z == 0 ? z0 : (z == 1 ? z1 : z2);
    for (uint32_t q = 0; q < log_ext; q++)
        if ((e >> q) & 1) acc = Fr::mul(acc, ld_fe(pow2tab + q));
    if (out29) st_f29(out29 + idx, Fr29::unpack(acc));
    else st_fe(out + idx, acc);
}
__global__ __launch_bounds__(256) void ntt_cm_transpose_kernel(const fe_t* in, fe_t* out, uint32_t log_n, uint32_t log_e, int to_natural) {
    const size_t j = (size_t)blockIdx.x * blockDim.x + threadIdx.x;
    if (j >> log_n) return;
    const uint32_t E = 1u << log_e;
    for (uint32_t b = 0; b < E; b++) {
        const size_t cm = ((size_t)b << log_n) + j, nat = (j << log_e) + b;
        if (to_natural) st_fe(out + nat, ld_fe(in + cm));
        else st_fe(out + cm, ld_fe(in + nat));
    }
}

struct NttPlan {
    uint32_t log_n = 0;
    int npass = 0;
    uint32_t log_radix[4] = {0, 0, 0, 0};
    fe_t* tw_inter[4] = {nullptr, nullptr, nullptr, nullptr};
    f29_t* stage29 = nullptr;
    fe_t n_inv;
};

struct CosetTables {
    f29_t* pre29 = nullptr;
    fe_t* inter = nullptr;
};
struct NttState {
    std::map<std::string, NttPlan*> plans;
    std::map<uint64_t, CosetTables> coset_tables;
    bool attrs_set = false;
};
static NttState& ntt_state() {
    Ctx* c = ctx();
    if (!c->ntt_state) c->ntt_state = new NttState();
    return *static_cast<NttState*>(c->ntt_state);
}
#define g_plans (ntt_state().plans)
#define g_coset_tables (ntt_state().coset_tables)

static uint32_t ntt_lds_stages(uint32_t log_r) { return log_r < 6 ? log_r : 6; }
static size_t ntt_lds_bytes(uint32_t log_tile, uint32_t log_r) { return 36u * ((size_t)1 << log_tile) + 36u * ((size_t)1 << ntt_lds_stages(log_r)); }
static fe_t ntt_domain_one() { return Fr::from_u64(32); }

static uint32_t ntt_max_radix() {
    static const uint32_t v = [] {
        const char* e = getenv("EZKL_NTT_MAXR");
        const int x = e ? atoi(e) : 0;
        return (uint32_t)(x >= 6 && x <= 11 ? x : 8);
    }();
    return v;
}
static void plan_radices(uint32_t log_n, NttPlan* p) {
    if (log_n <= NTT_LOG_SINGLE) {
        p->npass = 1;
        p->log_radix[0] = log_n;
        return;
    }
    const uint32_t maxr = ntt_max_radix();
    int np = (int)((log_n + maxr - 1) / maxr);
    if (np < 2) np = 2;
    if (np > 4) np = 4;
    p->npass = np;
    uint32_t base = log_n / np, extra = log_n % np;
    for (int i = 0; i < np; i++) p->log_radix[i] = base + ((uint32_t)i < extra ? 1 : 0);
}
static uint32_t pass_log_tile(uint32_t log_r) { return log_r >= 11 ? log_r : (log_r + 2 > NTT_LOG_TILE ? log_r + 2 : NTT_LOG_TILE); }
static void launch_pass(const PassArgs& a, uint32_t tiles, unsigned blocks_y, size_t lds, hipStream_t st) {
    if (a.npass > 1 && a.log_tile == 12) hipLaunchKernelGGL(ntt_pass_kernel<1024>, dim3(tiles, blocks_y), dim3(1024), lds, st, a);
    else if (a.npass > 1 && a.log_tile == 11) hipLaunchKernelGGL(ntt_pass_kernel<512>, dim3(tiles, blocks_y), dim3(512), lds, st, a);
    else hipLaunchKernelGGL(ntt_pass_kernel<256>, dim3(tiles, blocks_y), dim3(256), lds, st, a);
}
static int ntt_kernel_attrs() {
    bool& attr_set = ntt_state().attrs_set;
    if (!attr_set) {
        EZ_HIP(hipFuncSetAttribute((const void*)ntt_pass_kernel<256>, hipFuncAttributeMaxDynamicSharedMemorySize, 160 * 1024));
        EZ_HIP(hipFuncSetAttribute((const void*)ntt_pass_kernel<512>, hipFuncAttributeMaxDynamicSharedMemorySize, 160 * 1024));
        EZ_HIP(hipFuncSetAttribute((const void*)ntt_pass_kernel<1024>, hipFuncAttributeMaxDynamicSharedMemorySize, 160 * 1024));
        attr_set = true;
    }
    return EZKL_OK;
}

static int plan_get(Ctx* c, hipStream_t st, uint32_t log_n, const fe_t& omega, NttPlan** out) {
    std::string key((const char*)&omega, sizeof(fe_t));
    key.push_back((char)log_n);
    auto it = g_plans.find(key);
    if (it != g_plans.end()) { *out = it->second; return EZKL_OK; }
    NttPlan* p = new NttPlan();
    p->log_n = log_n;
    plan_radices(log_n, p);
    std::vector<fe_t> pow2(log_n ? log_n : 1);
    fe_t w = omega;
    for (uint32_t b = 0; b < log_n; b++) { pow2[b] = w; w = Fr::sqr(w); }
    p->n_inv = Fr::inv(Fr::from_u64((uint64_t)1 << log_n));
    fe_t* d_pow2 = nullptr;
    EZ_HIP(hipMalloc(&d_pow2, sizeof(fe_t) * pow2.size()));
    EZ_HIP(hipMemcpyAsync(d_pow2, pow2.data(), sizeof(fe_t) * pow2.size(), hipMemcpyHostToDevice, st));
    uint32_t log_m = log_n;
    const fe_t one = ntt_domain_one();
    {
        uint32_t maxlr = 0;
        for (int i = 0; i < p->npass; i++) maxlr = p->log_radix[i] > maxlr ? p->log_radix[i] : maxlr;
        const uint32_t cnt = 1u << maxlr;
        EZ_HIP(hipMalloc(&p->stage29, sizeof(f29_t) * cnt));
        hipLaunchKernelGGL(ntt_coset_table_kernel, dim3(cdiv(cnt, 256)), dim3(256), 0, st, (fe_t*)nullptr, p->stage29, cnt, 0u, log_n, 0u, 0, d_pow2, one, one, one);
    }
    for (int i = 0; i < p->npass; i++) {
        uint32_t lr = p->log_radix[i];
        if (i + 1 < p->npass) {
            uint32_t cnt = 1u << log_m;
            EZ_HIP(hipMalloc(&p->tw_inter[i], sizeof(fe_t) * (size_t)cnt));
            hipLaunchKernelGGL(ntt_twiddle_kernel, dim3(cdiv(cnt, 256)), dim3(256), 0, st, p->tw_inter[i], cnt,
                               (uint64_t)1 << (log_n - log_m), log_n, log_m - lr, 1, d_pow2, one);
        }
        log_m -= lr;
    }
    EZ_HIP(hipGetLastError());
    EZ_HIP(hipStreamSynchronize(st));
    EZ_HIP(hipFree(d_pow2));
    g_plans[key] = p;
    *out = p;
    return EZKL_OK;
}

static int ntt_run_chunk(Ctx* c, hipStream_t st, const fe_t* in, fe_t* out, uint32_t log_n, const fe_t& omega, bool inverse_scale,
                         size_t batch, size_t in_stride, size_t out_stride, uint32_t in_log_len, int coset_mode);

int ntt_run(Ctx* c, hipStream_t st, const fe_t* in, fe_t* out, uint32_t log_n, const fe_t& omega, bool inverse_scale,
            size_t batch, size_t in_stride, size_t out_stride, uint32_t in_log_len, int coset_mode) {
    if (log_n > 28 || in_log_len > log_n || batch == 0) return EZKL_ERR_INVALID;
    size_t group = ((size_t)4 << 30) / ((size_t)32 << log_n);
    if (group < 1) group = 1;
    if (group > 32768) group = 32768;
    for (size_t b0 = 0; b0 < batch; b0 += group) {
        size_t nb = batch - b0 < group ? batch - b0 : group;
        int rc = ntt_run_chunk(c, st, in + b0 * in_stride, out + b0 * out_stride, log_n, omega, inverse_scale, nb, in_stride, out_stride,
                               in_log_len, coset_mode);
        if (rc) return rc;
    }
    return EZKL_OK;
}

static int ntt_run_chunk(Ctx* c, hipStream_t st, const fe_t* in, fe_t* out, uint32_t log_n, const fe_t& omega, bool inverse_scale,
                         size_t batch, size_t in_stride, size_t out_stride, uint32_t in_log_len, int coset_mode) {
    NttPlan* p = nullptr;
    int rc = plan_get(c, st, log_n, omega, &p);
    if (rc) return rc;
    const size_t n = (size_t)1 << log_n;
    if ((rc = ntt_kernel_attrs())) return rc;
    fe_t* work = nullptr;
    if (p->npass > 1) {
        rc = arena_reserve(scratch_arena(c, st), batch * n * sizeof(fe_t), st, (void**)&work);
        if (rc) return rc;
    }
    const fe_t dom = ntt_domain_one();
    const fe_t zeta = Fr::mul(fr_const(FrConst::ZETA), dom), zeta2 = Fr::mul(fr_const(FrConst::ZETA2), dom);
    uint32_t log_m = log_n;
    hipEvent_t e0 = nullptr, e1 = nullptr;
    const char* tmode = getenv("EZKL_HIP_TIMING");
    const bool timed = !(tmode && !strcmp(tmode, "none"));
    if (timed) {
        rc = ev_pair(c, coset_mode ? "coset_ntt" : "ntt", &e0, &e1);
        if (rc) return rc;
        EZ_HIP(hipEventRecord(e0, st));
    }
    for (int i = 0; i < p->npass; i++) {
        PassArgs a;
        memset(&a, 0, sizeof a);
        const bool first = (i == 0), last = (i + 1 == p->npass);
        a.in = first ? in : work;
        a.in_stride = first ? in_stride : n;
        a.out = last ? out : work;
        a.out_stride = last ? out_stride : n;
        a.tw_inter = p->tw_inter[i];
        a.tw_stage29 = p->stage29;
        a.log_n = log_n;
        a.log_r = p->log_radix[i];
        a.lds_stages = ntt_lds_stages(a.log_r);
        a.log_m = log_m;
        a.log_tile = p->npass == 1 ? log_n : pass_log_tile(a.log_r);
        if (a.log_tile < a.log_r) a.log_tile = a.log_r;
        a.first = first;
        a.last = last;
        a.in_log_len = first ? in_log_len : log_n;
        a.coset_pre = (first && coset_mode == 1);
        a.npass = (uint32_t)p->npass;
        for (int q = 0; q < 4; q++) a.log_radix[q] = p->log_radix[q];
        a.zeta[0] = zeta;
        a.zeta[1] = zeta2;
        if (last) {
            uint32_t logC = a.log_tile - a.log_r;
            a.k1_major = (p->npass >= 2 && p->log_radix[0] >= logC) ? 1u : 0u;
            if (inverse_scale || coset_mode == 2) {
                a.post = 1;
                fe_t s = Fr::mul(inverse_scale || coset_mode == 2 ? p->n_inv : Fr::one(), dom);
                a.post_c[0] = s;
                a.post_c[1] = coset_mode == 2 ? Fr::mul(s, fr_const(FrConst::ZETA2)) : s;
                a.post_c[2] = coset_mode == 2 ? Fr::mul(s, fr_const(FrConst::ZETA)) : s;
            }
        }
        const uint32_t tiles = 1u << (log_n - a.log_tile);
        launch_pass(a, tiles, (unsigned)batch, ntt_lds_bytes(a.log_tile, a.log_r), st);
        log_m -= a.log_r;
    }
    EZ_HIP(hipGetLastError());
    if (timed) EZ_HIP(hipEventRecord(e1, st));
    if (work) return arena_done(scratch_arena(c, st), st);
    return EZKL_OK;
}



static int coset_tables_get(Ctx* c, hipStream_t st, NttPlan* p, uint32_t log_n, uint32_t log_ext, const fe_t& w_ext, CosetTables* out) {
    const uint64_t key = (uint64_t)log_n | ((uint64_t)log_ext << 8);
    auto it = g_coset_tables.find(key);
    if (it != g_coset_tables.end()) { *out = it->second; return EZKL_OK; }
    const uint32_t log_e = log_ext - log_n, lr = p->log_radix[0], log_s = log_n - lr;
    std::vector<fe_t> pow2(log_ext ? log_ext : 1);
    fe_t w = w_ext;
    for (uint32_t b = 0; b < log_ext; b++) { pow2[b] = w; w = Fr::sqr(w); }
    fe_t* d_pow2 = nullptr;
    EZ_HIP(hipMalloc(&d_pow2, sizeof(fe_t) * pow2.size()));
    EZ_HIP(hipMemcpyAsync(d_pow2, pow2.data(), sizeof(fe_t) * pow2.size(), hipMemcpyHostToDevice, st));
    CosetTables t;
    const fe_t one = ntt_domain_one(), zeta = Fr::mul(fr_const(FrConst::ZETA), one), zeta2 = Fr::mul(fr_const(FrConst::ZETA2), one);
    const size_t n_pre = (size_t)1 << (lr + log_e);
    EZ_HIP(hipMalloc(&t.pre29, sizeof(f29_t) * n_pre));
    hipLaunchKernelGGL(ntt_coset_table_kernel, dim3(cdiv(n_pre, 256)), dim3(256), 0, st, (fe_t*)nullptr, t.pre29, 1u << lr, log_e, log_ext, log_s, 0, d_pow2, one, zeta, zeta2);
    if (p->npass > 1) {
        const size_t n_int = (size_t)1 << log_ext;
        EZ_HIP(hipMalloc(&t.inter, sizeof(fe_t) * n_int));
        hipLaunchKernelGGL(ntt_coset_table_kernel, dim3(cdiv(n_int, 256)), dim3(256), 0, st, t.inter, (f29_t*)nullptr, 1u << log_n, log_e, log_ext, log_s, 1, d_pow2, one, zeta, zeta2);
    }
    EZ_HIP(hipGetLastError());
    EZ_HIP(hipStreamSynchronize(st));
    EZ_HIP(hipFree(d_pow2));
    g_coset_tables[key] = t;
    *out = t;
    return EZKL_OK;
}

static int coset_cm_chunk(Ctx* c, hipStream_t st, const fe_t* in, fe_t* out, uint32_t log_n, uint32_t log_ext, const fe_t& w_n, const fe_t& w_ext, size_t batch,
                          size_t in_stride, size_t out_stride, uint32_t first_coset, uint32_t log_count) {
    NttPlan* p = nullptr;
    int rc = plan_get(c, st, log_n, w_n, &p);
    if (rc) return rc;
    CosetTables ct;
    if ((rc = coset_tables_get(c, st, p, log_n, log_ext, w_ext, &ct))) return rc;
    const uint32_t log_e = log_ext - log_n;
    const size_t n = (size_t)1 << log_n, blocks = batch << log_count;
    if ((rc = ntt_kernel_attrs())) return rc;
    fe_t* work = nullptr;
    if (p->npass > 1) {
        rc = arena_reserve(scratch_arena(c, st), blocks * n * sizeof(fe_t), st, (void**)&work);
        if (rc) return rc;
    }
    uint32_t log_m = log_n;
    hipEvent_t e0, e1;
    if ((rc = ev_pair(c, "coset_ntt", &e0, &e1))) return rc;
    EZ_HIP(hipEventRecord(e0, st));
    for (int i = 0; i < p->npass; i++) {
        PassArgs a;
        memset(&a, 0, sizeof a);
        const bool first = (i == 0), last = (i + 1 == p->npass);
        a.in = first ? in : work;
        a.in_stride = first ? in_stride : n;
        a.out = last ? out : work;
        a.out_stride = last ? out_stride : n;
        a.tw_inter = first ? ct.inter : p->tw_inter[i];
        a.tw_stage29 = p->stage29;
        a.tw_pre29 = ct.pre29;
        a.log_n = log_n;
        a.log_r = p->log_radix[i];
        a.lds_stages = ntt_lds_stages(a.log_r);
        a.log_m = log_m;
        a.log_tile = p->npass == 1 ? log_n : pass_log_tile(a.log_r);
        if (a.log_tile < a.log_r) a.log_tile = a.log_r;
        a.first = first;
        a.last = last;
        a.in_log_len = log_n;
        a.npass = (uint32_t)p->npass;
        for (int q = 0; q < 4; q++) a.log_radix[q] = p->log_radix[q];
        a.cm = 1;
        a.cm_log_e = log_e;
        a.cm_first = first_coset;
        a.cm_log_cnt = log_count;
        if (last) {
            const uint32_t logC = a.log_tile - a.log_r;
            a.k1_major = (p->npass >= 2 && p->log_radix[0] >= logC) ? 1u : 0u;
        }
        const uint32_t tiles = 1u << (log_n - a.log_tile);
        launch_pass(a, tiles, (unsigned)blocks, ntt_lds_bytes(a.log_tile, a.log_r), st);
        log_m -= a.log_r;
    }
    EZ_HIP(hipGetLastError());
    EZ_HIP(hipEventRecord(e1, st));
    if (work) return arena_done(scratch_arena(c, st), st);
    return EZKL_OK;
}
int coset_cm_run(Ctx* c, hipStream_t st, const fe_t* in, fe_t* out, uint32_t log_n, uint32_t log_ext, const fe_t& w_n, const fe_t& w_ext, size_t batch,
                 size_t in_stride, size_t out_stride, uint32_t first_coset, uint32_t n_cosets) {
    if (log_ext > 28 || log_n > log_ext || log_ext - log_n > 6 || batch == 0) return EZKL_ERR_INVALID;
    const uint32_t E = 1u << (log_ext - log_n);
    if (n_cosets == 0) { first_coset = 0; n_cosets = E; }
    if ((n_cosets & (n_cosets - 1)) || first_coset + n_cosets > E) return EZKL_ERR_INVALID;
    uint32_t log_count = 0;
    while ((1u << log_count) < n_cosets) log_count++;
    size_t group = ((size_t)4 << 30) / ((size_t)32 << (log_n + log_count));
    if (group < 1) group = 1;
    if ((group << log_count) > 32768) group = 32768 >> log_count;
    for (size_t b0 = 0; b0 < batch; b0 += group) {
        const size_t nb = batch - b0 < group ? batch - b0 : group;
        int rc = coset_cm_chunk(c, st, in + b0 * in_stride, out + b0 * out_stride, log_n, log_ext, w_n, w_ext, nb, in_stride, out_stride, first_coset, log_count);
        if (rc) return rc;
    }
    return EZKL_OK;
}
int cm_transpose(Ctx* c, hipStream_t st, const fe_t* in, fe_t* out, uint32_t log_n, uint32_t log_e, bool to_natural) {
    (void)c;
    if (in == out || log_n + log_e > 28) return EZKL_ERR_INVALID;
    hipLaunchKernelGGL(ntt_cm_transpose_kernel, dim3(cdiv((size_t)1 << log_n, 256)), dim3(256), 0, st, in, out, log_n, log_e, to_natural ? 1 : 0);
// ... 6 lines not shown
```

### ezkl_amd/csrc/ubench.hip

```cpp
#include "common.hpp"
#include "curve.hpp"
#include "montmul29_gen.hpp"
#include "curve29.hpp"
#include "host64.hpp"
#include <string.h>
#include <vector>
#include <stdlib.h>

namespace ezkl {

template <int VARIANT>
__global__ __launch_bounds__(256) void ub_modmul_kernel(fe_t* io, int iters) {
    size_t i = (size_t)blockIdx.x * blockDim.x + threadIdx.x;
    fe_t a = ld_fe(io + i), b = a, c = Fr::add(a, a), d = c;
    b.v[0] ^= 5;  b = Fr::reduce_once(b);
    for (int k = 0; k < iters; k++) {
        if (VARIANT == 0) { a = Fr::mul(a, b); c = Fr::mul(c, d); b = Fr::mul(b, a); d = Fr::mul(d, c); }
        else if (VARIANT == 1) { a = Fr::mul_portable(a, b); c = Fr::mul_portable(c, d); b = Fr::mul_portable(b, a); d = Fr::mul_portable(d, c); }
        else { a = Fr::mul_inl(a, b); c = Fr::mul_inl(c, d); b = Fr::mul_inl(b, a); d = Fr::mul_inl(d, c); }
    }
    st_fe(io + i, Fr::add(Fr::add(a, b), Fr::add(c, d)));
}
__global__ __launch_bounds__(256) void ub_waveinv_kernel(fe_t* io, int iters) {
    size_t i = (size_t)blockIdx.x * blockDim.x + threadIdx.x;
// ... 95 lines not shown
__device__ __forceinline__ void mont_mul29_ref_fq(const uint32_t (&a)[9], const uint32_t (&b)[9], uint32_t (&r)[9]) {
    const uint32_t MASK = (1u << 29) - 1;
    uint32_t p[9];
    {
        uint64_t acc = 0; int bits = 0, w = 0;
        for (int i = 0; i < 9; i++) {
            while (bits < 29 && w < 8) { acc |= (uint64_t)FqP::MOD[w++] << bits; bits += 32; }
            p[i] = (uint32_t)acc & MASK; acc >>= 29; bits -= 29;
        }
    }
    uint32_t pinv = 1;
    for (int i = 0; i < 5; i++) pinv *= 2u - p[0] * pinv;
    pinv = (0u - pinv) & MASK;
    uint32_t m[9];
    uint64_t acc = 0;
    for (int k = 0; k < 17; k++) {
        for (int i = (k > 8 ? k - 8 : 0); i <= (k < 8 ? k : 8); i++) acc += (uint64_t)a[i] * b[k - i];
        for (int i = (k > 8 ? k - 8 : 0); i <= (k < 8 ? k : 8); i++)
            if (i < k || k >= 9) { if (i != k) acc += (uint64_t)m[i] * p[k - i]; }
        if (k < 9) {
            m[k] = ((uint32_t)acc * pinv) & MASK;
            acc += (uint64_t)m[k] * p[0];
        } else r[k - 9] = (uint32_t)acc & MASK;
        acc >>= 29;
    }
    r[8] = (uint32_t)acc;
}
__global__ __launch_bounds__(256) void ub_modmul29i_kernel(uint32_t* io, int iters, uint32_t* mismatches) {
    size_t t = (size_t)blockIdx.x * blockDim.x + threadIdx.x;
    uint32_t a[9], b[9], c[9], d[9], r[9];
    for (int i = 0; i < 9; i++) {
        uint32_t x = io[t * 8 + (i & 7)] * 2654435761u + i;
        a[i] = x & 0x1fffffffu; b[i] = (x >> 3) & 0x1fffffffu; c[i] = (x * 7u) & 0x1fffffffu; d[i] = (x * 13u) & 0x1fffffffu;
    }
    a[8] &= 0x3fffu; b[8] &= 0x3fffu; c[8] &= 0x3fffu; d[8] &= 0x3fffu;
    if (mismatches) {
        uint32_t want[9];
        bool bad = false;
        mont_mul29i_fq(a, b, r);
        mont_mul29_ref_fq(a, b, want);
        for (int i = 0; i < 9; i++) bad |= r[i] != want[i];
        mont_sqr29i_fq(c, r);
        mont_mul29_ref_fq(c, c, want);
        for (int i = 0; i < 9; i++) bad |= r[i] != want[i];
        mont_mul29i_fr(a, d, r);
        mont_mul29_fr(a, d, want);
        for (int i = 0; i < 9; i++) bad |= r[i] != want[i];
        if (bad) atomicAdd(mismatches, 1u);
    }
    for (int k = 0; k < iters; k++) {
        mont_mul29i_fq(a, b, r); for (int i = 0; i < 9; i++) a[i] = r[i];
        mont_mul29i_fq(c, d, r); for (int i = 0; i < 9; i++) c[i] = r[i];
        mont_mul29i_fq(b, a, r); for (int i = 0; i < 9; i++) b[i] = r[i];
        mont_mul29i_fq(d, c, r); for (int i = 0; i < 9; i++) d[i] = r[i];
    }
    uint32_t x = 0;
    for (int i = 0; i < 9; i++) x ^= a[i] ^ b[i] ^ c[i] ^ d[i];
    io[t * 8] = x;
}
__global__ __launch_bounds__(256) void ub_modmul29_kernel(uint32_t* io, int iters, uint32_t* mismatches) {
    size_t t = (size_t)blockIdx.x * blockDim.x + threadIdx.x;
    uint32_t a[9], b[9], c[9], d[9], r[9];
    for (int i = 0; i < 9; i++) {
        uint32_t x = io[t * 8 + (i & 7)] * 2654435761u + i;
        a[i] = x & 0x1fffffffu; b[i] = (x >> 3) & 0x1fffffffu; c[i] = (x * 7u) & 0x1fffffffu; d[i] = (x * 13u) & 0x1fffffffu;
    }
    a[8] &= 0x3fffu; b[8] &= 0x3fffu; c[8] &= 0x3fffu; d[8] &= 0x3fffu;
    if (mismatches) {
        uint32_t want[9];
        mont_mul29_fq(a, b, r);
        mont_mul29_ref_fq(a, b, want);
        bool bad = false;
        for (int i = 0; i < 9; i++) bad |= r[i] != want[i];
        if (bad) atomicAdd(mismatches, 1u);
    }
    for (int k = 0; k < iters; k++) {
        mont_mul29_fq(a, b, r); for (int i = 0; i < 9; i++) a[i] = r[i];
        mont_mul29_fq(c, d, r); for (int i = 0; i < 9; i++) c[i] = r[i];
        mont_mul29_fq(b, a, r); for (int i = 0; i < 9; i++) b[i] = r[i];
        mont_mul29_fq(d, c, r); for (int i = 0; i < 9; i++) d[i] = r[i];
    }
    uint32_t x = 0;
    for (int i = 0; i < 9; i++) x ^= a[i] ^ b[i] ^ c[i] ^ d[i];
    io[t * 8] = x;
}

template <int MODE>
__global__ __launch_bounds__(256) void ub_mix_kernel(uint64_t* io, int iters) {
    size_t i = (size_t)blockIdx.x * blockDim.x + threadIdx.x;
    uint64_t x = io[i];
    uint64_t a0 = x, a1 = x + 1, a2 = x + 2, a3 = x + 3, a4 = x + 4, a5 = x + 5, a6 = x + 6, a7 = x + 7;
    double d0 = (double)(x & 1023), d1 = d0 + 1, d2 = d0 + 2, d3 = d0 + 3, d4 = d0 + 4, d5 = d0 + 5, d6 = d0 + 6, d7 = d0 + 7;
    const double m = 1.0000001, q = 0.9999999;
    uint32_t mi = (uint32_t)x | 1u, qi = (uint32_t)(x >> 32) | 3u;
    for (int k = 0; k < iters; k++) {
        if (MODE == 0) {
            a0 = mad_wide(mi, (uint32_t)a0, a0); a1 = mad_wide(qi, (uint32_t)a1, a1); a2 = mad_wide(mi, (uint32_t)a2, a2); a3 = mad_wide(qi, (uint32_t)a3, a3);
            a4 = mad_wide(mi, (uint32_t)a4, a4); a5 = mad_wide(qi, (uint32_t)a5, a5); a6 = mad_wide(mi, (uint32_t)a6, a6); a7 = mad_wide(qi, (uint32_t)a7, a7);
        } else if (MODE == 1) {
            d0 = __builtin_fma(d0, m, q); d1 = __builtin_fma(d1, q, m); d2 = __builtin_fma(d2, m, q); d3 = __builtin_fma(d3, q, m);
            d4 = __builtin_fma(d4, m, q); d5 = __builtin_fma(d5, q, m); d6 = __builtin_fma(d6, m, q); d7 = __builtin_fma(d7, q, m);
        } else if (MODE == 2) {
            a0 = mad_wide(mi, (uint32_t)a0, a0); d4 = __builtin_fma(d4, m, q); a1 = mad_wide(qi, (uint32_t)a1, a1); d5 = __builtin_fma(d5, q, m);
            a2 = mad_wide(mi, (uint32_t)a2, a2); d6 = __builtin_fma(d6, m, q); a3 = mad_wide(qi, (uint32_t)a3, a3); d7 = __builtin_fma(d7, q, m);
        } else if (MODE == 3) {
            asm volatile("v_lshl_add_u64 %0, %0, 0, %1\n\tv_lshl_add_u64 %1, %1, 0, %2\n\tv_lshl_add_u64 %2, %2, 0, %3\n\tv_lshl_add_u64 %3, %3, 0, %4\n\t"
                         "v_lshl_add_u64 %4, %4, 0, %5\n\tv_lshl_add_u64 %5, %5, 0, %6\n\tv_lshl_add_u64 %6, %6, 0, %7\n\tv_lshl_add_u64 %7, %7, 0, %0"
                         : "+v"(a0), "+v"(a1), "+v"(a2), "+v"(a3), "+v"(a4), "+v"(a5), "+v"(a6), "+v"(a7));
        } else {
            asm volatile("v_add_f64 %0, %0, %8\n\tv_add_f64 %1, %1, %9\n\tv_add_f64 %2, %2, %8\n\tv_add_f64 %3, %3, %9\n\t"
                         "v_add_f64 %4, %4, %8\n\tv_add_f64 %5, %5, %9\n\tv_add_f64 %6, %6, %8\n\tv_add_f64 %7, %7, %9"
                         : "+v"(d0), "+v"(d1), "+v"(d2), "+v"(d3), "+v"(d4), "+v"(d5), "+v"(d6), "+v"(d7) : "v"(m), "v"(q));
        }
    }
    io[i] = a0 ^ a1 ^ a2 ^ a3 ^ a4 ^ a5 ^ a6 ^ a7 ^ (uint64_t)(d0 + d1 + d2 + d3 + d4 + d5 + d6 + d7);
}

struct Dfma52 {
    static constexpr uint64_t M52 = (1ull << 52) - 1;
    EZ_HD static constexpr uint64_t limb(int i) {
        uint64_t v = 0;
        for (int b = 0; b < 52; b++) {
            const int bit = 52 * i + b;
            if (bit < 256 && ((FqP::MOD[bit >> 5] >> (bit & 31)) & 1u)) v |= 1ull << b;
        }
        return v;
    }
    EZ_HD static constexpr uint64_t pinv() {
        uint64_t x = 1;
        for (int i = 0; i < 6; i++) x *= 2 - limb(0) * x;
        return (0 - x) & M52;
    }
};
__device__ __forceinline__ void dfma_hilo(double a, double b, uint64_t& hi_raw, uint64_t& lo_raw) {
    const double C1 = 0x1p104, C2 = 0x1p104 + 0x1p52;
    const double h = __builtin_fma(a, b, C1);
    const double s = C2 - h;
    const double l = __builtin_fma(a, b, s);
    hi_raw = (uint64_t)__double_as_longlong(h);
    lo_raw = (uint64_t)__double_as_longlong(l);
}
__device__ __forceinline__ void mont_mul52_dfma_fq(const double (&a)[5], const double (&b)[5], double (&r)[5]) {
    constexpr uint64_t HI_PAT = 0x4670000000000000ull, LO_PAT = 0x4330000000000000ull, M52 = Dfma52::M52;
    double m[5];
    double pd[5];
#pragma unroll
    for (int i = 0; i < 5; i++) pd[i] = (double)Dfma52::limb(i);
    const double pinv = (double)Dfma52::pinv();
    uint64_t carry = 0, nxt = 0;
#pragma unroll
    for (int k = 0; k < 10; k++) {
        uint64_t acc = carry + nxt, hi, lo;
        nxt = 0;
        int cnt = 0;
#pragma unroll
        for (int i = 0; i < 5; i++) {
            const int j = k - i;
            if (j < 0 || j > 4) continue;
            dfma_hilo(a[i], b[j], hi, lo);
            acc += lo; nxt += hi; cnt++;
            if (i < k && i < 5 && k < 5) {}
        }
#pragma unroll
        for (int i = 0; i < 5; i++) {
            const int j = k - i;
            if (j < 0 || j > 4) continue;
// ... 181 lines not shown
        EZ_HIP(hipFree(buf));
        const double per_thread = (is_mm || !strcmp(which, "addsub")) ? 4.0 * iters : 8.0 * iters;
        *out = per_thread * (double)nthreads / (ms * 1e-3);
        return EZKL_OK;
    }
    if (!strcmp(which, "waveinv")) {
        const int threads = 256, blocks = c->num_cus * 16, iters = 16;
        const size_t nthreads = (size_t)threads * blocks;
        void* buf = nullptr;
        EZ_HIP(hipMalloc(&buf, nthreads * sizeof(fe_t)));
        std::vector<fe_t> init(nthreads);
        for (size_t t = 0; t < nthreads; t++) { init[t] = Fr::one(); init[t].v[0] = (uint32_t)(t * 2654435761u) | 1u; init[t].v[7] = 0; }
        EZ_HIP(hipMemcpy(buf, init.data(), nthreads * sizeof(fe_t), hipMemcpyHostToDevice));
        hipEvent_t e0, e1;
        EZ_HIP(hipEventCreate(&e0)); EZ_HIP(hipEventCreate(&e1));
        float ms = 0;
        for (int rep = 0; rep < 2; rep++) {
            EZ_HIP(hipEventRecord(e0, st));
            hipLaunchKernelGGL(ub_waveinv_kernel, dim3(blocks), dim3(threads), 0, st, (fe_t*)buf, iters);
            EZ_HIP(hipEventRecord(e1, st));
            EZ_HIP(hipEventSynchronize(e1));
            EZ_HIP(hipEventElapsedTime(&ms, e0, e1));
        }
        (void)hipEventDestroy(e0); (void)hipEventDestroy(e1);
        (void)hipFree(buf);
        *out = (double)nthreads * iters / (ms * 1e-3);
        return EZKL_OK;
    }
    if (!strncmp(which, "mix_", 4)) {
        void* buf = nullptr;
        int blocks = c->num_cus * 16;
        if (const char* o = strstr(which, "_o")) blocks = c->num_cus * atoi(o + 2);
        const size_t nthreads = (size_t)blocks * threads;
        EZ_HIP(hipMalloc(&buf, nthreads * 8));
        EZ_HIP(hipMemsetAsync(buf, 0x11, nthreads * 8, st));
        const int iters = 4096;
        for (int rep = 0; rep < 2; rep++) {
            EZ_HIP(hipEventRecord(e0, st));
            if (!strncmp(which, "mix_mad", 7)) hipLaunchKernelGGL(ub_mix_kernel<0>, dim3(blocks), dim3(threads), 0, st, (uint64_t*)buf, iters);
            else if (!strncmp(which, "mix_dfma", 8)) hipLaunchKernelGGL(ub_mix_kernel<1>, dim3(blocks), dim3(threads), 0, st, (uint64_t*)buf, iters);
            else if (!strncmp(which, "mix_both", 8)) hipLaunchKernelGGL(ub_mix_kernel<2>, dim3(blocks), dim3(threads), 0, st, (uint64_t*)buf, iters);
            else if (!strncmp(which, "mix_add64", 9)) hipLaunchKernelGGL(ub_mix_kernel<3>, dim3(blocks), dim3(threads), 0, st, (uint64_t*)buf, iters);
            else hipLaunchKernelGGL(ub_mix_kernel<4>, dim3(blocks), dim3(threads), 0, st, (uint64_t*)buf, iters);
            EZ_HIP(hipEventRecord(e1, st));
            EZ_HIP(hipStreamSynchronize(st));
            EZ_HIP(hipEventElapsedTime(&ms, e0, e1));
        }
        EZ_HIP(hipFree(buf));
        *out = 8.0 * iters * (double)nthreads / (ms * 1e-3);
        return EZKL_OK;
    }
    if (!strncmp(which, "dfma52", 6)) {
        void* buf = nullptr;
        uint32_t* mis = nullptr;
        const bool chk = strstr(which, "check") != nullptr;
        const int iters = chk ? 1 : 256;
        int blocks = c->num_cus * 16;
        if (const char* o = strstr(which, "_o")) blocks = c->num_cus * atoi(o + 2);
        const size_t nthreads = (size_t)blocks * threads;
        EZ_HIP(hipMalloc(&buf, nthreads * 32));
        EZ_HIP(hipMalloc((void**)&mis, 4));
        {
            std::vector<uint32_t> h(nthreads * 8);
            uint64_t x = 0x9e3779b97f4a7c15ull;
            for (auto& w : h) { x ^= x << 13; x ^= x >> 7; x ^= x << 17; w = (uint32_t)(x >> 16); }
            EZ_HIP(hipMemcpyAsync(buf, h.data(), nthreads * 32, hipMemcpyHostToDevice, st));
            EZ_HIP(hipStreamSynchronize(st));
        }
        EZ_HIP(hipMemsetAsync(mis, 0, 4, st));
        for (int rep = 0; rep < 2; rep++) {
            EZ_HIP(hipEventRecord(e0, st));
            hipLaunchKernelGGL(ub_dfma52_kernel, dim3(blocks), dim3(threads), 0, st, (uint32_t*)buf, iters, chk ? mis : nullptr);
            EZ_HIP(hipEventRecord(e1, st));
            EZ_HIP(hipStreamSynchronize(st));
            EZ_HIP(hipEventElapsedTime(&ms, e0, e1));
        }
        uint32_t hm = 0;
        EZ_HIP(hipMemcpy(&hm, mis, 4, hipMemcpyDeviceToHost));
        EZ_HIP(hipFree(buf));
        EZ_HIP(hipFree(mis));
        *out = chk ? (double)hm : 4.0 * iters * (double)nthreads / (ms * 1e-3);
        return EZKL_OK;
    }
    if (!strncmp(which, "modmul29", 8)) {
        void* buf = nullptr;
        uint32_t* mis = nullptr;
        EZ_HIP(hipMalloc(&buf, nthreads * 32));
        EZ_HIP(hipMalloc((void**)&mis, 4));
        EZ_HIP(hipMemsetAsync(buf, 0x5b, nthreads * 32, st));
        EZ_HIP(hipMemsetAsync(mis, 0, 4, st));
        const bool chk = strstr(which, "check") != nullptr;
        const int iters = chk ? 1 : 256;
        int blocks = c->num_cus * 16;
        if (const char* o = strstr(which, "_o")) blocks = c->num_cus * atoi(o + 2);
        const size_t nthreads = (size_t)blocks * threads;
        for (int rep = 0; rep < 2; rep++) {
            EZ_HIP(hipEventRecord(e0, st));
            if (!strncmp(which, "modmul29i", 9)) hipLaunchKernelGGL(ub_modmul29i_kernel, dim3(blocks), dim3(threads), 0, st, (uint32_t*)buf, iters, chk ? mis : nullptr);
            else hipLaunchKernelGGL(ub_modmul29_kernel, dim3(blocks), dim3(threads), 0, st, (uint32_t*)buf, iters, chk ? mis : nullptr);
            EZ_HIP(hipEventRecord(e1, st));
            EZ_HIP(hipStreamSynchronize(st));
            EZ_HIP(hipEventElapsedTime(&ms, e0, e1));
        }
        uint32_t hm = 0;
        EZ_HIP(hipMemcpy(&hm, mis, 4, hipMemcpyDeviceToHost));
        EZ_HIP(hipFree(buf));
        EZ_HIP(hipFree(mis));
        *out = chk ? (double)hm : 4.0 * iters * (double)nthreads / (ms * 1e-3);
        return EZKL_OK;
    }
    if (!strncmp(which, "ecadd", 5)) {
        const int iters = atoi(which + 5);
        const char mode = which[strlen(which) - 1];
        const bool full = mode == 'f';
        const int eb = full ? c->num_cus * 4 : mode == 'h' ? c->num_cus * 4 : mode == 'q' ? c->num_cus : 1, et = full ? 256 : 64;
        void* buf = nullptr;
        const size_t cnt = (size_t)eb * et + 1;
        EZ_HIP(hipMalloc(&buf, cnt * sizeof(g1x_t)));
        EZ_HIP(hipMemsetAsync(buf, 0, cnt * sizeof(g1x_t), st));
        {
            std::vector<g1x_t> h(cnt);
            g1x_t g;
            g.x = Fq::one(); g.y = Fq::add(Fq::one(), Fq::one()); g.zz = Fq::one(); g.zzz = Fq::one();
            for (size_t i = 0; i < cnt; i++) h[i] = g;
            for (size_t i = 0; i + 1 < cnt; i += 2) h[i] = g1x_double(g);
            EZ_HIP(hipMemcpyAsync(buf, h.data(), cnt * sizeof(g1x_t), hipMemcpyHostToDevice, st));
            EZ_HIP(hipStreamSynchronize(st));
        }
        for (int rep = 0; rep < 4; rep++) {
            EZ_HIP(hipEventRecord(e0, st));
            if (which[5] == 't') hipLaunchKernelGGL(ub_ectree_kernel, dim3(eb), dim3(64), 0, st, (g1x_t*)buf);
            else if (which[5] == 'u') hipLaunchKernelGGL(ub_ectree_u_kernel, dim3(eb), dim3(64), 0, st, (g1x_t*)buf);
            else if (which[5] == 'v') hipLaunchKernelGGL(ub_ectree_v_kernel, dim3(eb), dim3(64), 0, st, (g1x_t*)buf, 0u);
            else if (which[5] == 'x') hipLaunchKernelGGL(ub_ectree_v_kernel, dim3(eb), dim3(64), 0, st, (g1x_t*)buf, 64u);
            else hipLaunchKernelGGL(ub_ecadd_kernel, dim3(eb), dim3(et), 0, st, (g1x_t*)buf, iters);
            EZ_HIP(hipEventRecord(e1, st));
            EZ_HIP(hipStreamSynchronize(st));
            EZ_HIP(hipEventElapsedTime(&ms, e0, e1));
        }
        EZ_HIP(hipFree(buf));
        *out = ms * 1e3;
        return EZKL_OK;
    }
    if (!strcmp(which, "coopcheck")) {
        const Bases* dummy = nullptr; (void)dummy;
        g1a_t* pts = nullptr;
        uint32_t* o = nullptr;
        EZ_HIP(hipMalloc(&pts, 512 * sizeof(g1a_t)));
        EZ_HIP(hipMalloc(&o, 64 * (160 + 128 + 72 + 36) * 4));
        EZ_HIP(hipMemsetAsync(o, 0, 64 * (160 + 128 + 72 + 36) * 4, st));
        {
            std::vector<g1a_t> h(512);
            h64::aff g;
            memset(&g, 0, sizeof g);
            h64::fe one; { uint32_t w[8]; for (int q = 0; q < 8; q++) w[q] = Fq::one().v[q]; one = h64::from32(w); }
            g.x = one; g.y = h64::add(one, one);
            h64::xyzz acc = h64::from_affine(g), G = acc;
            h64::fe k261; { uint32_t w[8]; for (int q = 0; q < 8; q++) w[q] = Fq29C::R261_32[q]; k261 = h64::from32(w); }
            for (int i = 0; i < 512; i++) {
                h64::aff a = h64::to_affine(acc);
                h64::fe tx = h64::mul(a.x, k261), ty = h64::mul(a.y, k261);
                memcpy(&h[i].x, &tx, 32); memcpy(&h[i].y, &ty, 32);
                acc = h64::add(acc, G);
                acc = h64::add(acc, G);
                acc = h64::add(acc, G);
            }
            EZ_HIP(hipMemcpy(pts, h.data(), 512 * sizeof(g1a_t), hipMemcpyHostToDevice));
        }
        hipLaunchKernelGGL(ub_coopcheck_kernel, dim3(1), dim3(64), 0, st, pts, o);
        EZ_HIP(hipStreamSynchronize(st));
        std::vector<uint32_t> h(64 * (160 + 128 + 72 + 36));
        EZ_HIP(hipMemcpy(h.data(), o, h.size() * 4, hipMemcpyDeviceToHost));
        uint32_t mask = 0;
        {
            uint32_t* o2 = nullptr;
            EZ_HIP(hipMalloc(&o2, 256 * 216 * 4));
            std::vector<uint32_t> h2(256 * 216);
            for (int ident = 0; ident < 2; ident++) {
                hipLaunchKernelGGL(ub_coopcheck2_kernel, dim3(1), dim3(256), 0, st, pts, o2, ident);
                EZ_HIP(hipStreamSynchronize(st));
                EZ_HIP(hipMemcpy(h2.data(), o2, h2.size() * 4, hipMemcpyDeviceToHost));
// ... 118 lines not shown
```

### ezkl_amd/lib.py

```python
import ctypes as C
import os

_HERE = os.path.dirname(os.path.abspath(__file__))
_LIB = None

SYMBOLS = [
    "ezkl_hip_init", "ezkl_hip_contexts_configure", "ezkl_hip_context_count", "ezkl_hip_set_context", "ezkl_hip_context_device", "ezkl_hip_memcpy_peer", "ezkl_hip_warmup", "ezkl_hip_device_count", "ezkl_hip_mem_info", "ezkl_hip_pool_stats", "ezkl_hip_pool_trim", "ezkl_hip_synchronize", "ezkl_hip_stream_create", "ezkl_hip_stream_synchronize", "ezkl_hip_stream_destroy", "ezkl_hip_context_stream", "ezkl_hip_strerror",
    "ezkl_hip_last_hip_error", "ezkl_hip_version", "ezkl_hip_enabled", "ezkl_hip_malloc", "ezkl_hip_free", "ezkl_hip_memcpy_h2d",
    "ezkl_hip_memcpy_d2h", "ezkl_hip_bases_upload", "ezkl_hip_bases_prepare", "ezkl_hip_bases_free", "ezkl_hip_bases_len", "ezkl_hip_bases_generate",
    "ezkl_hip_bases_download", "ezkl_hip_bases_from_scalars", "ezkl_hip_bases_downsize", "ezkl_hip_msm_g2", "ezkl_hip_msm_g1",
    "ezkl_hip_msm_g1_dev", "ezkl_hip_msm_g1_start_dev", "ezkl_hip_msm_g1_finish", "ezkl_hip_msm_g1_batch", "ezkl_hip_msm_g1_batch_dev", "ezkl_hip_msm_g1_batch_small_dev", "ezkl_hip_g1_add_affine", "ezkl_hip_ntt", "ezkl_hip_ntt_dev",
    "ezkl_hip_coset_ntt_batch", "ezkl_hip_coset_ntt_dev", "ezkl_hip_coeff_to_cosets_dev", "ezkl_hip_coeff_to_cosets_range_dev", "ezkl_hip_cosets_transpose_dev", "ezkl_hip_vec_op_dev", "ezkl_hip_vec_scale_dev", "ezkl_hip_permutation_sigma_dev", "ezkl_hip_vec_fill_dev", "ezkl_hip_host_malloc", "ezkl_hip_host_free", "ezkl_hip_upload_commit_batch", "ezkl_hip_upload_begin", "ezkl_hip_upload_begin_fmt", "ezkl_hip_upload_wait", "ezkl_hip_upload_commit", "ezkl_hip_upload_end", "ezkl_hip_msm_batch_begin", "ezkl_hip_msm_batch_push_dev", "ezkl_hip_msm_batch_push_many_dev", "ezkl_hip_msm_batch_finish", "ezkl_hip_eval_poly_batch_dev", "ezkl_hip_lincomb_dev", "ezkl_hip_kate_division_dev", "ezkl_hip_chacha20_fr_dev",
    "ezkl_hip_divide_by_vanishing_dev", "ezkl_hip_prefix_scan_dev", "ezkl_hip_eval_poly_dev", "ezkl_hip_lookup_multiplicity_dev", "ezkl_hip_lookup_multiplicity_acc_dev", "ezkl_hip_lookup_multiplicity_batch_dev", "ezkl_hip_batch_invert_dev", "ezkl_hip_eval_h_dev", "ezkl_hip_eval_h_check", "ezkl_hip_eval_h_source", "ezkl_hip_eval_h_schedule", "ezkl_hip_eval_h_prepare", "ezkl_hip_eval_h_jit_stats", "ezkl_hip_eval_check_dev", "ezkl_hip_eval_check_source", "ezkl_hip_lookup_missing_rows_dev", "ezkl_hip_copy_check_dev", "ezkl_hip_set_async", "ezkl_hip_stream_wait_library",
    "ezkl_hip_last_kernel_ms", "ezkl_hip_kernel_ms_stats", "ezkl_hip_ubench",
    "ezkl_hip_witness_plan_upload", "ezkl_hip_witness_plan_free", "ezkl_hip_witness_plan_info", "ezkl_hip_witness_run_dev", "ezkl_hip_witness_last_error",
    "ezkl_hip_comm_available", "ezkl_hip_comm_unique_id", "ezkl_hip_comm_init", "ezkl_hip_comm_info", "ezkl_hip_comm_destroy", "ezkl_hip_comm_allgather_dev",
    "ezkl_hip_comm_fold_points", "ezkl_hip_comm_broadcast_host", "ezkl_hip_comm_alltoall_dev", "ezkl_hip_comm_allgather_host", "ezkl_hip_comm_alltoallv_dev", "ezkl_hip_comm_stats", "ezkl_hip_comm_selftest",
]


class EzklHipError(RuntimeError):
    def __init__(self, code, what):
        self.code = code
        msg = load().ezkl_hip_strerror(code).decode() if _LIB is not None else "library not loaded"
        super().__init__("%s failed: %d (%s)" % (what, code, msg))


def lib_path():
    return os.environ.get("EZKL_HIP_LIB") or os.path.join(_HERE, "libezkl_hip.so")


def load():
    global _LIB
    if _LIB is None:
        path = lib_path()
        if not os.path.exists(path):
            raise RuntimeError("libezkl_hip.so missing at %s -- build it with `make -C ezkl_amd/csrc` "
                               "(there is no CPU fallback)" % path)
        lib = C.CDLL(path)
        lib.ezkl_hip_strerror.restype = C.c_char_p
        lib.ezkl_hip_version.restype = C.c_char_p
        lib.ezkl_hip_witness_last_error.restype = C.c_char_p
        lib.ezkl_hip_bases_len.restype = C.c_size_t
        _LIB = lib
    return _LIB


def check(rc, what):
    if rc != 0:
        raise EzklHipError(rc, what)
```

### include/ezkl_hip.h

```cpp
#ifndef EZKL_HIP_H
#define EZKL_HIP_H
#include <stddef.h>
#include <stdint.h>
#ifdef __cplusplus
extern "C" {
#endif

#define EZKL_OK 0
#define EZKL_ERR_NO_DEVICE (-1)
#define EZKL_ERR_HIP (-2)
#define EZKL_ERR_INVALID (-3)
#define EZKL_ERR_NOMEM (-4)
#define EZKL_ERR_UNSUPPORTED (-5)
#define EZKL_ERR_TIMEOUT (-7)
#define EZKL_ERR_BUSY (-6)



typedef struct ezkl_bases_s* ezkl_bases_t;

int ezkl_hip_init(int device);
int ezkl_hip_contexts_configure(int n_contexts, const int* devices);
int ezkl_hip_context_count(void);
int ezkl_hip_set_context(int index);
// ... 2 lines not shown
int ezkl_hip_warmup(void);
int ezkl_hip_device_count(void);
int ezkl_hip_mem_info(size_t* free_bytes, size_t* total_bytes);
int ezkl_hip_pool_stats(size_t out[4]);
int ezkl_hip_pool_trim(void);
int ezkl_hip_synchronize(void);
int ezkl_hip_stream_create(void** out_stream);
int ezkl_hip_stream_synchronize(void* stream);
int ezkl_hip_stream_destroy(void* stream);
int ezkl_hip_context_stream(void** out_stream);
int ezkl_hip_set_async(int on, int* previous);
int ezkl_hip_stream_wait_library(void* stream);
const char* ezkl_hip_strerror(int code);
int ezkl_hip_last_hip_error(void);
const char* ezkl_hip_version(void);
int ezkl_hip_enabled(uint32_t k);

int ezkl_hip_malloc(void** dptr, size_t bytes);
int ezkl_hip_free(void* dptr);
int ezkl_hip_memcpy_h2d(void* dst_dev, const void* src_host, size_t bytes);
int ezkl_hip_host_malloc(void** host_ptr, size_t bytes);
int ezkl_hip_host_free(void* host_ptr);
int ezkl_hip_memcpy_d2h(void* dst_host, const void* src_dev, size_t bytes);

int ezkl_hip_bases_upload(const void* affine_pts, size_t n, ezkl_bases_t* out_handle);
int ezkl_hip_bases_prepare(ezkl_bases_t h);
int ezkl_hip_bases_free(ezkl_bases_t h);
size_t ezkl_hip_bases_len(ezkl_bases_t h);
int ezkl_hip_bases_generate(uint64_t seed, size_t first, size_t n, ezkl_bases_t* out_handle);
int ezkl_hip_bases_download(ezkl_bases_t h, void* out_host );
int ezkl_hip_bases_from_scalars(const void* base_point, const void* scalars_dev, size_t n, ezkl_bases_t* out_handle);
int ezkl_hip_bases_downsize(ezkl_bases_t g, uint32_t new_k, ezkl_bases_t* out_g, ezkl_bases_t* out_g_lagrange);
int ezkl_hip_msm_g2(const void* points_affine, const void* scalars, size_t n, void* out_affine);
int ezkl_hip_msm_g1(ezkl_bases_t h, const void* scalars, size_t n, void* out_affine);
int ezkl_hip_msm_g1_dev(ezkl_bases_t h, size_t base_offset, const void* scalars_dev, size_t n,
                        void* out_affine, void* stream);
int ezkl_hip_msm_g1_batch(ezkl_bases_t h, const void* const* scalars, size_t batch, size_t n, void* out_affine);
int ezkl_hip_msm_g1_start_dev(ezkl_bases_t h, size_t base_offset, const void* scalars_dev, size_t n, int* token);
int ezkl_hip_msm_g1_finish(int token, void* out_affine);
int ezkl_hip_msm_g1_batch_dev(ezkl_bases_t h, size_t base_offset, const void* const* scalars_dev, size_t batch, size_t n,
                              void* out_affine, void* stream);
int ezkl_hip_msm_g1_batch_small_dev(ezkl_bases_t h, size_t base_offset, const void* const* scalars_dev, size_t batch, size_t n,
                                    void* out_affine, void* stream);
int ezkl_hip_upload_commit_batch(ezkl_bases_t h, const void* const* host_cols, void* const* dev_cols, size_t batch, size_t n,
                                 const void* const* tail_rows, size_t tail_start, size_t tail_count, size_t commit_first, size_t commit_count,
                                 void* out_affine);
typedef struct ezkl_upload_s* ezkl_upload_t;
int ezkl_hip_upload_begin(const void* const* host_cols, void* const* dev_cols, size_t batch, size_t n, const void* const* tail_rows,
                          size_t tail_start, size_t tail_count, ezkl_upload_t* out_upload);
#define EZKL_COLUMN_FP 0
#define EZKL_COLUMN_INT64 1
#define EZKL_COLUMN_INT128 2
#define EZKL_COLUMN_DEVICE_FP 3
int ezkl_hip_upload_begin_fmt(const void* const* host_cols, const uint8_t* formats, void* const* dev_cols, size_t batch, size_t n,
                              const void* const* tail_rows, size_t tail_start, size_t tail_count, ezkl_upload_t* out_upload);
int ezkl_hip_upload_wait(ezkl_upload_t upload, size_t column, void* stream);
int ezkl_hip_upload_commit(ezkl_upload_t upload, ezkl_bases_t h, size_t commit_first, size_t commit_count, void* out_affine);
int ezkl_hip_upload_end(ezkl_upload_t upload);
typedef struct ezkl_wplan_s* ezkl_wplan_t;
int ezkl_hip_witness_plan_upload(const void* blob, size_t len, ezkl_wplan_t* out_plan);
int ezkl_hip_witness_plan_free(ezkl_wplan_t plan);
int ezkl_hip_witness_plan_info(ezkl_wplan_t plan, uint32_t out[8]);
int ezkl_hip_witness_run_dev(ezkl_wplan_t plan, const int64_t* inputs_host, size_t n_inputs, void* const* advice_cols_dev, void* outputs_host,
                             uint64_t status[4], void* stream);
const char* ezkl_hip_witness_last_error(void);
typedef struct ezkl_msm_batch_s* ezkl_msm_batch_t;
int ezkl_hip_msm_batch_begin(ezkl_bases_t h, size_t base_offset, size_t n, ezkl_msm_batch_t* out_batch);
int ezkl_hip_msm_batch_push_dev(ezkl_msm_batch_t batch, const void* scalars_dev);
int ezkl_hip_msm_batch_push_many_dev(ezkl_msm_batch_t batch, const void* const* scalars_dev, size_t count);
int ezkl_hip_msm_batch_finish(ezkl_msm_batch_t batch, void* out_affine, size_t capacity);
int ezkl_hip_g1_add_affine(const void* a, const void* b, void* out);

int ezkl_hip_ntt(void* data, uint32_t log_n, const void* omega, int inverse);
int ezkl_hip_ntt_dev(void* data_dev, uint32_t log_n, const void* omega, int inverse,
                     size_t batch, size_t stride_elems, void* stream);
int ezkl_hip_coset_ntt_batch(const void* const* in, void* const* out, size_t batch,
                             uint32_t log_n, uint32_t log_n_ext, int inverse);
int ezkl_hip_coset_ntt_dev(const void* in_dev, void* out_dev, size_t batch, size_t in_stride_elems,
                           size_t out_stride_elems, uint32_t log_n, uint32_t log_n_ext, int inverse, void* stream);

int ezkl_hip_coeff_to_cosets_dev(const void* in_dev, void* out_dev, size_t batch, size_t in_stride_elems, size_t out_stride_elems,
                                 uint32_t log_n, uint32_t log_n_ext, void* stream);
int ezkl_hip_cosets_transpose_dev(const void* in_dev, void* out_dev, uint32_t log_n, uint32_t log_n_ext, int to_natural, void* stream);
int ezkl_hip_coeff_to_cosets_range_dev(const void* in_dev, void* out_dev, size_t batch, size_t in_stride_elems, size_t out_stride_elems,
                                       uint32_t log_n, uint32_t log_n_ext, uint32_t first_coset, uint32_t n_cosets, void* stream);

#define EZKL_VEC_ADD 0
#define EZKL_VEC_SUB 1
#define EZKL_VEC_MUL 2
int ezkl_hip_vec_op_dev(int op, const void* a_dev, const void* b_dev, void* out_dev, size_t n, void* stream);
int ezkl_hip_vec_scale_dev(const void* a_dev, const void* scalar_host, void* out_dev, size_t n, void* stream);
int ezkl_hip_vec_fill_dev(void* out_dev, const void* value_host, size_t n, void* stream);
int ezkl_hip_permutation_sigma_dev(const void* next_dev, const void* omega_col_dev, const void* delta_pows_dev, uint32_t n_columns, uint32_t log_n,
                                   void* out_dev, void* stream);
int ezkl_hip_divide_by_vanishing_dev(void* a_dev, uint32_t k, uint32_t ext_k, void* stream);
int ezkl_hip_prefix_scan_dev(int op, int exclusive, const void* in_dev, void* out_dev, size_t n, void* stream);
int ezkl_hip_lookup_multiplicity_dev(const void* const* inputs_dev, uint32_t n_inputs, const void* table_dev, uint32_t n_rows,
                                     uint32_t usable_rows, void* m_out_dev, uint32_t* out_missing, void* stream);
int ezkl_hip_lookup_multiplicity_acc_dev(const void* const* inputs_dev, uint32_t n_inputs, const void* table_dev, uint32_t n_rows,
                                         uint32_t usable_rows, void* m_out_dev, void* missing_dev, void* stream);
int ezkl_hip_lookup_multiplicity_batch_dev(const void* const* inputs_dev, const uint32_t* input_lookup, uint32_t n_inputs, const void* const* tables_dev,
                                           uint32_t n_lookups, uint32_t n_rows, uint32_t usable_rows, void* const* m_outs_dev, void* missing_dev, void* stream);
int ezkl_hip_eval_poly_dev(const void* coeffs_dev, size_t n, const void* x_host, void* out_host, void* stream);
int ezkl_hip_eval_poly_batch_dev(const void* const* coeffs_dev, const void* xs_host, uint32_t m, size_t n, void* out_host, void* stream);
int ezkl_hip_kate_division_dev(const void* a_dev, const void* z_host, void* out_dev, size_t n, void* stream);
int ezkl_hip_lincomb_dev(const void* const* inputs_dev, const void* coeffs_host, uint32_t m, void* out_dev, size_t n, int accumulate,
                         void* stream);
int ezkl_hip_chacha20_fr_dev(const void* key32, uint64_t stream_id, size_t first, void* out_dev, size_t n, void* stream);
int ezkl_hip_batch_invert_dev(void* a_dev, size_t n, void* stream);

enum { EZKL_OP_ADD = 0, EZKL_OP_SUB, EZKL_OP_MUL, EZKL_OP_SQUARE, EZKL_OP_DOUBLE, EZKL_OP_NEGATE,
       EZKL_OP_STORE, EZKL_OP_HORNER_STEP  };
enum { EZKL_SRC_CONST = 0, EZKL_SRC_INTERMEDIATE, EZKL_SRC_COLUMN, EZKL_SRC_CHALLENGE, EZKL_SRC_PREVIOUS };
typedef struct {
    const uint32_t* code;       uint32_t n_instr;  uint32_t n_intermediates;
    const void* constants;      uint32_t n_constants;
    const int32_t* rotations;   uint32_t n_rotations;
    const void* const* columns; uint32_t n_columns;
    const void* challenges;     uint32_t n_challenges;
    uint32_t k, ext_k;
} ezkl_program_t;
int ezkl_hip_eval_h_dev(const ezkl_program_t* prog, void* out_dev, void* stream);
int ezkl_hip_eval_h_check(const ezkl_program_t* prog);
int ezkl_hip_eval_h_source(const ezkl_program_t* prog, char* out, size_t cap, size_t* len);
int ezkl_hip_eval_h_schedule(const ezkl_program_t* prog, uint32_t* out_code);
int ezkl_hip_eval_h_prepare(const ezkl_program_t* prog);
int ezkl_hip_eval_h_jit_stats(uint64_t* compiled, uint64_t* from_disk, uint64_t* memory_hits);

typedef struct { uint32_t kind, index, sub, row; } ezkl_check_record_t;
int ezkl_hip_eval_check_dev(const ezkl_program_t* prog, const uint32_t* check_slots, uint32_t n_checks, uint32_t row_lo, uint32_t row_hi, void* records_dev,
                            uint32_t cap, void* counters_dev, void* stream);
int ezkl_hip_eval_check_source(const ezkl_program_t* prog, const uint32_t* check_slots, uint32_t n_checks, char* out, size_t cap, size_t* len);
int ezkl_hip_lookup_missing_rows_dev(const void* const* inputs_dev, const uint32_t* input_lookup, uint32_t n_inputs, const void* const* tables_dev,
                                     uint32_t n_lookups, uint32_t n_rows, uint32_t usable_rows, void* records_dev, uint32_t cap, void* counters_dev,
                                     void* stream);
int ezkl_hip_copy_check_dev(const void* const* cols_dev, uint32_t m, const void* next_dev, uint32_t log_n, void* records_dev, uint32_t cap, void* counters_dev,
                            void* stream);

int ezkl_hip_comm_unique_id(void* out128);
int ezkl_hip_comm_init(const void* id128, int world, int rank);
int ezkl_hip_comm_info(int* world, int* rank);
int ezkl_hip_comm_destroy(void);
int ezkl_hip_comm_allgather_dev(void* buf_dev, size_t total_bytes);
int ezkl_hip_comm_fold_points(void* points_host, uint32_t count);
int ezkl_hip_comm_broadcast_host(void* buf_host, size_t bytes, int root);
int ezkl_hip_comm_alltoall_dev(const void* send_dev, const size_t* send_off, const size_t* send_len, void* recv_dev, const size_t* recv_off,
                               const size_t* recv_len);

int ezkl_hip_comm_allgather_host(void* buf_host, size_t bytes_per_rank);
int ezkl_hip_comm_available(void);
typedef struct { int peer; void* ptr; size_t bytes; } ezkl_comm_seg_t;
int ezkl_hip_comm_alltoallv_dev(const ezkl_comm_seg_t* sends, size_t n_sends, const ezkl_comm_seg_t* recvs, size_t n_recvs);
int ezkl_hip_comm_stats(uint64_t out[8], int reset);
int ezkl_hip_comm_selftest(void);

int ezkl_hip_last_kernel_ms(const char* which, float* out_ms);
int ezkl_hip_kernel_ms_stats(const char* which, double* sum_ms, uint64_t* count, int reset);
int ezkl_hip_ubench(const char* which, double* out);

#ifdef __cplusplus
}
#endif
#endif
```

Measured before the change: 796.0 million pts/s.

## Use Shoup-style precomputed-quotient twiddle multiplication in NTT stages

Adds a constant-multiplier modular multiply (mulc) for the Fr field that pairs each twiddle with a precomputed quotient-helper value, replacing full Montgomery multiplication in NTT butterflies. Twiddle tables become pairs (tw29_t), doubling table memory and load traffic, in exchange for fewer reduction multiplies per butterfly. It also adds a table-download API and a microbenchmark with correctness checks. The headline MSM metric should be largely unaffected; the NTT throughput is the main target.

New measurement: 795.4 million pts/s (median of 2 runs). No clear change (-0.1%).

```diff
diff --git a/ezkl_amd/backend.py b/ezkl_amd/backend.py
--- a/ezkl_amd/backend.py
+++ b/ezkl_amd/backend.py
@@ -399,6 +399,15 @@
     _l.check(_l.load().ezkl_hip_coeff_to_cosets_range_dev(_vp(in_ptr), _vp(out_ptr), C.c_size_t(batch), C.c_size_t(1 << k), C.c_size_t(n_cosets << k),
                                                            C.c_uint32(k), C.c_uint32(ext_k), C.c_uint32(first_coset), C.c_uint32(n_cosets), _stream_ptr(stream)),
              "ezkl_hip_coeff_to_cosets_range_dev")
+
+
+def ntt_tables_download(k, ext_k=0):
+    cnt = C.c_size_t(0)
+    cap = 1 << (min(k, 11) + (ext_k - k if ext_k else 0))
+    out = np.zeros((cap, 2, 9), np.uint32)
+    _l.check(_l.load().ezkl_hip_ntt_tables_download(C.c_uint32(k), C.c_uint32(ext_k), out.ctypes.data_as(C.c_void_p), C.c_size_t(cap), C.byref(cnt)),
+             "ezkl_hip_ntt_tables_download")
+    return out[:cnt.value]
 
 
 def cosets_transpose_dev(in_ptr, out_ptr, k, ext_k, to_natural=True, stream=None):
diff --git a/ezkl_amd/csrc/capi.hip b/ezkl_amd/csrc/capi.hip
--- a/ezkl_amd/csrc/capi.hip
+++ b/ezkl_amd/csrc/capi.hip
@@ -874,6 +874,11 @@
     if (rc) return rc;
     return finish(c, st, stream);
 }
+int ezkl_hip_ntt_tables_download(uint32_t log_n, uint32_t log_n_ext, void* out, size_t capacity, size_t* count) {
+    if (!out || !count || log_n == 0 || log_n > 28 || (log_n_ext && (log_n_ext < log_n || log_n_ext > 28 || log_n_ext - log_n > 6))) return EZKL_ERR_INVALID;
+    EZ_CTX(c);
+    return ntt_tables_download(c, c->stream, log_n, log_n_ext, domain_omega(log_n, false), domain_omega(log_n_ext ? log_n_ext : log_n, false), out, capacity, count);
+}
 int ezkl_hip_cosets_transpose_dev(const void* in, void* out, uint32_t log_n, uint32_t log_n_ext, int to_natural, void* stream) {
     if (!in || !out || in == out || log_n > log_n_ext || log_n_ext > 28) return EZKL_ERR_INVALID;
     EZ_CTX(c);
diff --git a/ezkl_amd/csrc/common.hpp b/ezkl_amd/csrc/common.hpp
--- a/ezkl_amd/csrc/common.hpp
+++ b/ezkl_amd/csrc/common.hpp
@@ -98,6 +98,7 @@
 
 int ntt_run(Ctx* c, hipStream_t st, const fe_t* in, fe_t* out, uint32_t log_n, const fe_t& omega, bool inverse_scale,
             size_t batch, size_t in_stride, size_t out_stride, uint32_t in_log_len, int coset_mode);
+int ntt_tables_download(Ctx* c, hipStream_t st, uint32_t log_n, uint32_t log_ext, const fe_t& w_n, const fe_t& w_ext, void* out, size_t capacity, size_t* count);
 int coset_cm_run(Ctx* c, hipStream_t st, const fe_t* in, fe_t* out, uint32_t log_n, uint32_t log_ext, const fe_t& w_n, const fe_t& w_ext, size_t batch,
                  size_t in_stride, size_t out_stride, uint32_t first_coset = 0, uint32_t n_cosets = 0);
 int cm_transpose(Ctx* c, hipStream_t st, const fe_t* in, fe_t* out, uint32_t log_n, uint32_t log_e, bool to_natural);
diff --git a/ezkl_amd/csrc/field29.hpp b/ezkl_amd/csrc/field29.hpp
--- a/ezkl_amd/csrc/field29.hpp
+++ b/ezkl_amd/csrc/field29.hpp
@@ -68,6 +68,33 @@
         mont_mul2add29_fq(a.v, b.v, c.v, d.v, r.v);
         return r;
     }
+    EZ_D static f29_t mulc(const f29_t& v, const f29_t& w, const f29_t& wq) {
+        static_assert(!IS_FQ, "generated for Fr only");
+        f29_t r;
+        mulc29_fr(v.v, w.v, wq.v, r.v);
+        return r;
+    }
+    EZ_D static void mulc_pair(const f29_t& W, f29_t& w, f29_t& wq) {
+        f29_t one = zero();
+        one.v[0] = 1;
+        w = cond_sub<0>(mul(W, one));
+        uint64_t acc = 0;
+        uint32_t t[9];
+#pragma unroll
+        for (int k = 0; k < 9; k++) {
+#pragma unroll
+            for (int i = 0; i <= k; i++) acc += (uint64_t)W.v[i] * C::PINV261[k - i];
+            t[k] = (uint32_t)acc & M29;
+            acc >>= 29;
+        }
+        uint32_t carry = 1;
+#pragma unroll
+        for (int k = 0; k < 9; k++) {
+            const uint32_t x = (M29 - t[k]) + carry;
+            wq.v[k] = x & M29;
+            carry = x >> 29;
+        }
+    }
     EZ_D static f29_t mul_cold(const f29_t& a, const f29_t& b) {
         u32x9 x, y;
 #pragma unroll
@@ -185,6 +212,9 @@
     }
 };
 
+struct tw29_t {
+    f29_t w, q;
+};
 typedef Field29<Fq29C, true> Fq29;
 typedef Field29<Fr29C, false> Fr29;
 
diff --git a/ezkl_amd/csrc/montmul29_gen.hpp b/ezkl_amd/csrc/montmul29_gen.hpp
--- a/ezkl_amd/csrc/montmul29_gen.hpp
+++ b/ezkl_amd/csrc/montmul29_gen.hpp
@@ -23,6 +23,8 @@
         {0x1c1815c8u, 0x17dcfa49u, 0x1c6ae587u, 0x0956e978u, 0x13d1343fu, 0x0925f9fau, 0x1ac8f5f7u, 0x0d1ece5fu, 0x1e7cdd8cu},
     };
     static constexpr uint32_t R261_32[8] = {0x157ccc21u, 0x4e8384ebu, 0x0ce148c3u, 0xfb90a602u, 0x819caa36u, 0x5301fa84u, 0x563d4475u, 0x0dc83629u};
+    static constexpr uint32_t NEGP[9] = {0x078302b9u, 0x1efb9f49u, 0x038d5cb0u, 0x1d2add2fu, 0x0a7a2687u, 0x1d24bf3fu, 0x1f591ebeu, 0x11a3d9cbu, 0x1fcf9bb1u};
+    static constexpr uint32_t PINV261[9] = {0x1b799c77u, 0x016fc3e8u, 0x0d654d9eu, 0x030535c2u, 0x0257f612u, 0x1a17f3e6u, 0x0e509d40u, 0x090dceeeu, 0x100a85ddu};
 };
 struct Fr29C {
     static constexpr uint32_t P[9] = {0x10000001u, 0x1f0fac9fu, 0x0e5c2450u, 0x07d090f3u, 0x1585d283u, 0x02db40c0u, 0x00a6e141u, 0x0e5c2634u, 0x0030644eu};
@@ -44,6 +46,8 @@
         {0x1ffffff8u, 0x07829b03u, 0x0d1edd78u, 0x017b7864u, 0x13d16be6u, 0x0925f9fau, 0x1ac8f5f7u, 0x0d1ece5fu, 0x1e7cdd8cu},
     };
     static constexpr uint32_t R261_32[8] = {0x8fffff57u, 0x2fd4e156u, 0xa494b01au, 0x75bba827u, 0x819caa80u, 0x5301fa84u, 0x563d4475u, 0x0dc83629u};
+    static constexpr uint32_t NEGP[9] = {0x0fffffffu, 0x00f05360u, 0x11a3dbafu, 0x182f6f0cu, 0x0a7a2d7cu, 0x1d24bf3fu, 0x1f591ebeu, 0x11a3d9cbu, 0x1fcf9bb1u};
+    static constexpr uint32_t PINV261[9] = {0x10000001u, 0x08f05360u, 0x05bb930fu, 0x12f36967u, 0x1dc6e9a7u, 0x13ebb37cu, 0x19347195u, 0x1c5e4f97u, 0x0d8c07d0u};
 };
 __device__ __forceinline__ void mont_mul29_fq(const uint32_t (&a)[9], const uint32_t (&b)[9], uint32_t (&r)[9]) {
     asm("s_mov_b32 s16, 0x187cfd47\n\t"
@@ -1875,4 +1879,200 @@
         : [a0] "v"(a[0]), [a1] "v"(a[1]), [a2] "v"(a[2]), [a3] "v"(a[3]), [a4] "v"(a[4]), [a5] "v"(a[5]), [a6] "v"(a[6]), [a7] "v"(a[7]), [a8] "v"(a[8]), [b0] "v"(b[0]), [b1] "v"(b[1]), [b2] "v"(b[2]), [b3] "v"(b[3]), [b4] "v"(b[4]), [b5] "v"(b[5]), [b6] "v"(b[6]), [b7] "v"(b[7]), [b8] "v"(b[8])
         : "v16", "v17", "v18", "v19", "s16", "s17", "s18", "s19", "s20", "s21", "s22", "s23", "s24", "s25", "s26", "vcc");
 }
+__device__ __forceinline__ void mulc29_fr(const uint32_t (&v)[9], const uint32_t (&w)[9], const uint32_t (&wq)[9], uint32_t (&r)[9]) {
+    uint32_t q[9];
+    for (int i = 0; i < 9; i++) r[i] = wq[i];
+    asm("s_mov_b32 s16, 0x0fffffff\n\t"
+        "s_mov_b32 s17, 0x00f05360\n\t"
+        "s_mov_b32 s18, 0x11a3dbaf\n\t"
+        "s_mov_b32 s19, 0x182f6f0c\n\t"
+        "s_mov_b32 s20, 0x0a7a2d7c\n\t"
+        "s_mov_b32 s21, 0x1d24bf3f\n\t"
+        "s_mov_b32 s22, 0x1f591ebe\n\t"
+        "s_mov_b32 s23, 0x11a3d9cb\n\t"
+        "s_mov_b32 s24, 0x1fcf9bb1\n\t"
+        "s_mov_b32 s26, 0x1fffffff\n\t"
+        "v_mad_u64_u32 v[16:17], vcc, %[r0], %[v7], 0\n\t"
+        "v_mad_u64_u32 v[16:17], vcc, %[r1], %[v6], v[16:17]\n\t"
+        "v_mad_u64_u32 v[16:17], vcc, %[r2], %[v5], v[16:17]\n\t"
+        "v_mad_u64_u32 v[16:17], vcc, %[r3], %[v4], v[16:17]\n\t"
+        "v_mad_u64_u32 v[16:17], vcc, %[r4], %[v3], v[16:17]\n\t"
+        "v_mad_u64_u32 v[16:17], vcc, %[r5], %[v2], v[16:17]\n\t"
+        "v_mad_u64_u32 v[16:17], vcc, %[r6], %[v1], v[16:17]\n\t"
+        "v_mad_u64_u32 v[16:17], vcc, %[r7], %[v0], v[16:17]\n\t"
+        "v_lshrrev_b64 v[16:17], 29, v[16:17]\n\t"
+        "v_mad_u64_u32 v[16:17], vcc, %[r0], %[v8], v[16:17]\n\t"
+        "v_mad_u64_u32 v[16:17], vcc, %[r1], %[v7], v[16:17]\n\t"
+        "v_mad_u64_u32 v[16:17], vcc, %[r2], %[v6], v[16:17]\n\t"
+        "v_mad_u64_u32 v[16:17], vcc, %[r3], %[v5], v[16:17]\n\t"
+        "v_mad_u64_u32 v[16:17], vcc, %[r4], %[v4], v[16:17]\n\t"
+        "v_mad_u64_u32 v[16:17], vcc, %[r5], %[v3], v[16:17]\n\t"
+        "v_mad_u64_u32 v[16:17], vcc, %[r6], %[v2], v[16:17]\n\t"
+        "v_mad_u64_u32 v[16:17], vcc, %[r7], %[v1], v[16:17]\n\t"
+        "v_mad_u64_u32 v[16:17], vcc, %[r8], %[v0], v[16:17]\n\t"
+        "v_lshrrev_b64 v[16:17], 29, v[16:17]\n\t"
+        "v_mad_u64_u32 v[16:17], vcc, %[r1], %[v8], v[16:17]\n\t"
+        "v_mad_u64_u32 v[16:17], vcc, %[r2], %[v7], v[16:17]\n\t"
+        "v_mad_u64_u32 v[16:17], vcc, %[r3], %[v6], v[16:17]\n\t"
+        "v_mad_u64_u32 v[16:17], vcc, %[r4], %[v5], v[16:17]\n\t"
+        "v_mad_u64_u32 v[16:17], vcc, %[r5], %[v4], v[16:17]\n\t"
+        "v_mad_u64_u32 v[16:17], vcc, %[r6], %[v3], v[16:17]\n\t"
+        "v_mad_u64_u32 v[16:17], vcc, %[r7], %[v2], v[16:17]\n\t"
+        "v_mad_u64_u32 v[16:17], vcc, %[r8], %[v1], v[16:17]\n\t"
+        "v_and_b32 %[q0], s26, v16\n\t"
+        "v_lshrrev_b64 v[16:17], 29, v[16:17]\n\t"
+        "v_mad_u64_u32 v[18:19], vcc, %[w0], %[v0], 0\n\t"
+        "v_mad_u64_u32 v[16:17], vcc, %[r2], %[v8], v[16:17]\n\t"
+        "v_mad_u64_u32 v[18:19], vcc, %[q0], s16, v[18:19]\n\t"
+        "v_mad_u64_u32 v[16:17], vcc, %[r3], %[v7], v[16:17]\n\t"
+        "v_and_b32 %[r0], s26, v18\n\t"
+        "v_mad_u64_u32 v[16:17], vcc, %[r4], %[v6], v[16:17]\n\t"
+        "v_lshrrev_b64 v[18:19], 29, v[18:19]\n\t"
+        "v_mad_u64_u32 v[16:17], vcc, %[r5], %[v5], v[16:17]\n\t"
+        "v_mad_u64_u32 v[16:17], vcc, %[r6], %[v4], v[16:17]\n\t"
+        "v_mad_u64_u32 v[16:17], vcc, %[r7], %[v3], v[16:17]\n\t"
+        "v_mad_u64_u32 v[16:17], vcc, %[r8], %[v2], v[16:17]\n\t"
+        "v_and_b32 %[q1], s26, v16\n\t"
+        "v_lshrrev_b64 v[16:17], 29, v[16:17]\n\t"
+        "v_mad_u64_u32 v[18:19], vcc, %[w0], %[v1], v[18:19]\n\t"
+        "v_mad_u64_u32 v[16:17], vcc, %[r3], %[v8], v[16:17]\n\t"
+        "v_mad_u64_u32 v[18:19], vcc, %[w1], %[v0], v[18:19]\n\t"
+        "v_mad_u64_u32 v[16:17], vcc, %[r4], %[v7], v[16:17]\n\t"
+        "v_mad_u64_u32 v[18:19], vcc, %[q0], s17, v[18:19]\n\t"
+        "v_mad_u64_u32 v[16:17], vcc, %[r5], %[v6], v[16:17]\n\t"
+        "v_mad_u64_u32 v[18:19], vcc, %[q1], s16, v[18:19]\n\t"
+        "v_mad_u64_u32 v[16:17], vcc, %[r6], %[v5], v[16:17]\n\t"
+        "v_and_b32 %[r1], s26, v18\n\t"
+        "v_mad_u64_u32 v[16:17], vcc, %[r7], %[v4], v[16:17]\n\t"
+        "v_lshrrev_b64 v[18:19], 29, v[18:19]\n\t"
+        "v_mad_u64_u32 v[16:17], vcc, %[r8], %[v3], v[16:17]\n\t"
+        "v_and_b32 %[q2], s26, v16\n\t"
+        "v_lshrrev_b64 v[16:17], 29, v[16:17]\n\t"
+        "v_mad_u64_u32 v[18:19], vcc, %[w0], %[v2], v[18:19]\n\t"
+        "v_mad_u64_u32 v[16:17], vcc, %[r4], %[v8], v[16:17]\n\t"
+        "v_mad_u64_u32 v[18:19], vcc, %[w1], %[v1], v[18:19]\n\t"
+        "v_mad_u64_u32 v[16:17], vcc, %[r5], %[v7], v[16:17]\n\t"
+        "v_mad_u64_u32 v[18:19], vcc, %[w2], %[v0], v[18:19]\n\t"
+        "v_mad_u64_u32 v[16:17], vcc, %[r6], %[v6], v[16:17]\n\t"
+        "v_mad_u64_u32 v[18:19], vcc, %[q0], s18, v[18:19]\n\t"
+        "v_mad_u64_u32 v[16:17], vcc, %[r7], %[v5], v[16:17]\n\t"
+        "v_mad_u64_u32 v[18:19], vcc, %[q1], s17, v[18:19]\n\t"
+        "v_mad_u64_u32 v[16:17], vcc, %[r8], %[v4], v[16:17]\n\t"
+        "v_mad_u64_u32 v[18:19], vcc, %[q2], s16, v[18:19]\n\t"
+        "v_and_b32 %[q3], s26, v16\n\t"
+        "v_and_b32 %[r2], s26, v18\n\t"
+        "v_lshrrev_b64 v[16:17], 29, v[16:17]\n\t"
+        "v_lshrrev_b64 v[18:19], 29, v[18:19]\n\t"
+        "v_mad_u64_u32 v[18:19], vcc, %[w0], %[v3], v[18:19]\n\t"
+        "v_mad_u64_u32 v[16:17], vcc, %[r5], %[v8], v[16:17]\n\t"
+        "v_mad_u64_u32 v[18:19], vcc, %[w1], %[v2], v[18:19]\n\t"
+        "v_mad_u64_u32 v[16:17], vcc, %[r6], %[v7], v[16:17]\n\t"
+        "v_mad_u64_u32 v[18:19], vcc, %[w2], %[v1], v[18:19]\n\t"
+        "v_mad_u64_u32 v[16:17], vcc, %[r7], %[v6], v[16:17]\n\t"
+        "v_mad_u64_u32 v[18:19], vcc, %[w3], %[v0], v[18:19]\n\t"
+        "v_mad_u64_u32 v[16:17], vcc, %[r8], %[v5], v[16:17]\n\t"
+        "v_mad_u64_u32 v[18:19], vcc, %[q0], s19, v[18:19]\n\t"
+        "v_and_b32 %[q4], s26, v16\n\t"
+        "v_mad_u64_u32 v[18:19], vcc, %[q1], s18, v[18:19]\n\t"
+        "v_lshrrev_b64 v[16:17], 29, v[16:17]\n\t"
+        "v_mad_u64_u32 v[18:19], vcc, %[q2], s17, v[18:19]\n\t"
+        "v_mad_u64_u32 v[18:19], vcc, %[q3], s16, v[18:19]\n\t"
+        "v_and_b32 %[r3], s26, v18\n\t"
+        "v_lshrrev_b64 v[18:19], 29, v[18:19]\n\t"
+        "v_mad_u64_u32 v[18:19], vcc, %[w0], %[v4], v[18:19]\n\t"
+        "v_mad_u64_u32 v[16:17], vcc, %[r6], %[v8], v[16:17]\n\t"
+        "v_mad_u64_u32 v[18:19], vcc, %[w1], %[v3], v[18:19]\n\t"
+        "v_mad_u64_u32 v[16:17], vcc, %[r7], %[v7], v[16:17]\n\t"
+        "v_mad_u64_u32 v[18:19], vcc, %[w2], %[v2], v[18:19]\n\t"
+        "v_mad_u64_u32 v[16:17], vcc, %[r8], %[v6], v[16:17]\n\t"
+        "v_mad_u64_u32 v[18:19], vcc, %[w3], %[v1], v[18:19]\n\t"
+        "v_and_b32 %[q5], s26, v16\n\t"
+        "v_mad_u64_u32 v[18:19], vcc, %[w4], %[v0], v[18:19]\n\t"
+        "v_lshrrev_b64 v[16:17], 29, v[16:17]\n\t"
+        "v_mad_u64_u32 v[18:19], vcc, %[q0], s20, v[18:19]\n\t"
+        "v_mad_u64_u32 v[18:19], vcc, %[q1], s19, v[18:19]\n\t"
+        "v_mad_u64_u32 v[18:19], vcc, %[q2], s18, v[18:19]\n\t"
+        "v_mad_u64_u32 v[18:19], vcc, %[q3], s17, v[18:19]\n\t"
+        "v_mad_u64_u32 v[18:19], vcc, %[q4], s16, v[18:19]\n\t"
+        "v_and_b32 %[r4], s26, v18\n\t"
+        "v_lshrrev_b64 v[18:19], 29, v[18:19]\n\t"
+        "v_mad_u64_u32 v[18:19], vcc, %[w0], %[v5], v[18:19]\n\t"
+        "v_mad_u64_u32 v[16:17], vcc, %[r7], %[v8], v[16:17]\n\t"
+        "v_mad_u64_u32 v[18:19], vcc, %[w1], %[v4], v[18:19]\n\t"
+        "v_mad_u64_u32 v[16:17], vcc, %[r8], %[v7], v[16:17]\n\t"
+        "v_mad_u64_u32 v[18:19], vcc, %[w2], %[v3], v[18:19]\n\t"
+        "v_and_b32 %[q6], s26, v16\n\t"
+        "v_mad_u64_u32 v[18:19], vcc, %[w3], %[v2], v[18:19]\n\t"
+        "v_lshrrev_b64 v[16:17], 29, v[16:17]\n\t"
+        "v_mad_u64_u32 v[18:19], vcc, %[w4], %[v1], v[18:19]\n\t"
+        "v_mad_u64_u32 v[18:19], vcc, %[w5], %[v0], v[18:19]\n\t"
+        "v_mad_u64_u32 v[18:19], vcc, %[q0], s21, v[18:19]\n\t"
+        "v_mad_u64_u32 v[18:19], vcc, %[q1], s20, v[18:19]\n\t"
+        "v_mad_u64_u32 v[18:19], vcc, %[q2], s19, v[18:19]\n\t"
+        "v_mad_u64_u32 v[18:19], vcc, %[q3], s18, v[18:19]\n\t"
+        "v_mad_u64_u32 v[18:19], vcc, %[q4], s17, v[18:19]\n\t"
+        "v_mad_u64_u32 v[18:19], vcc, %[q5], s16, v[18:19]\n\t"
+        "v_and_b32 %[r5], s26, v18\n\t"
+        "v_lshrrev_b64 v[18:19], 29, v[18:19]\n\t"
+        "v_mad_u64_u32 v[18:19], vcc, %[w0], %[v6], v[18:19]\n\t"
+        "v_mad_u64_u32 v[16:17], vcc, %[r8], %[v8], v[16:17]\n\t"
+        "v_mad_u64_u32 v[18:19], vcc, %[w1], %[v5], v[18:19]\n\t"
+        "v_and_b32 %[q7], s26, v16\n\t"
+        "v_mad_u64_u32 v[18:19], vcc, %[w2], %[v4], v[18:19]\n\t"
+        "v_lshrrev_b64 v[16:17], 29, v[16:17]\n\t"
+        "v_mad_u64_u32 v[18:19], vcc, %[w3], %[v3], v[18:19]\n\t"
+        "v_mov_b32 %[q8], v16\n\t"
+        "v_mad_u64_u32 v[18:19], vcc, %[w4], %[v2], v[18:19]\n\t"
+        "v_mad_u64_u32 v[18:19], vcc, %[w5], %[v1], v[18:19]\n\t"
+        "v_mad_u64_u32 v[18:19], vcc, %[w6], %[v0], v[18:19]\n\t"
+        "v_mad_u64_u32 v[18:19], vcc, %[q0], s22, v[18:19]\n\t"
+        "v_mad_u64_u32 v[18:19], vcc, %[q1], s21, v[18:19]\n\t"
+        "v_mad_u64_u32 v[18:19], vcc, %[q2], s20, v[18:19]\n\t"
+        "v_mad_u64_u32 v[18:19], vcc, %[q3], s19, v[18:19]\n\t"
+        "v_mad_u64_u32 v[18:19], vcc, %[q4], s18, v[18:19]\n\t"
+        "v_mad_u64_u32 v[18:19], vcc, %[q5], s17, v[18:19]\n\t"
+        "v_mad_u64_u32 v[18:19], vcc, %[q6], s16, v[18:19]\n\t"
+        "v_and_b32 %[r6], s26, v18\n\t"
+        "v_lshrrev_b64 v[18:19], 29, v[18:19]\n\t"
+        "v_mad_u64_u32 v[18:19], vcc, %[w0], %[v7], v[18:19]\n\t"
+        "v_mad_u64_u32 v[18:19], vcc, %[w1], %[v6], v[18:19]\n\t"
+        "v_mad_u64_u32 v[18:19], vcc, %[w2], %[v5], v[18:19]\n\t"
+        "v_mad_u64_u32 v[18:19], vcc, %[w3], %[v4], v[18:19]\n\t"
+        "v_mad_u64_u32 v[18:19], vcc, %[w4], %[v3], v[18:19]\n\t"
+        "v_mad_u64_u32 v[18:19], vcc, %[w5], %[v2], v[18:19]\n\t"
+        "v_mad_u64_u32 v[18:19], vcc, %[w6], %[v1], v[18:19]\n\t"
+        "v_mad_u64_u32 v[18:19], vcc, %[w7], %[v0], v[18:19]\n\t"
+        "v_mad_u64_u32 v[18:19], vcc, %[q0], s23, v[18:19]\n\t"
+        "v_mad_u64_u32 v[18:19], vcc, %[q1], s22, v[18:19]\n\t"
+        "v_mad_u64_u32 v[18:19], vcc, %[q2], s21, v[18:19]\n\t"
+        "v_mad_u64_u32 v[18:19], vcc, %[q3], s20, v[18:19]\n\t"
+        "v_mad_u64_u32 v[18:19], vcc, %[q4], s19, v[18:19]\n\t"
+        "v_mad_u64_u32 v[18:19], vcc, %[q5], s18, v[18:19]\n\t"
+        "v_mad_u64_u32 v[18:19], vcc, %[q6], s17, v[18:19]\n\t"
+        "v_mad_u64_u32 v[18:19], vcc, %[q7], s16, v[18:19]\n\t"
+        "v_and_b32 %[r7], s26, v18\n\t"
+        "v_lshrrev_b64 v[18:19], 29, v[18:19]\n\t"
+        "v_mad_u64_u32 v[18:19], vcc, %[w0], %[v8], v[18:19]\n\t"
+        "v_mad_u64_u32 v[18:19], vcc, %[w1], %[v7], v[18:19]\n\t"
+        "v_mad_u64_u32 v[18:19], vcc, %[w2], %[v6], v[18:19]\n\t"
+        "v_mad_u64_u32 v[18:19], vcc, %[w3], %[v5], v[18:19]\n\t"
+        "v_mad_u64_u32 v[18:19], vcc, %[w4], %[v4], v[18:19]\n\t"
+        "v_mad_u64_u32 v[18:19], vcc, %[w5], %[v3], v[18:19]\n\t"
+        "v_mad_u64_u32 v[18:19], vcc, %[w6], %[v2], v[18:19]\n\t"
+        "v_mad_u64_u32 v[18:19], vcc, %[w7], %[v1], v[18:19]\n\t"
+        "v_mad_u64_u32 v[18:19], vcc, %[w8], %[v0], v[18:19]\n\t"
+        "v_mad_u64_u32 v[18:19], vcc, %[q0], s24, v[18:19]\n\t"
+        "v_mad_u64_u32 v[18:19], vcc, %[q1], s23, v[18:19]\n\t"
+        "v_mad_u64_u32 v[18:19], vcc, %[q2], s22, v[18:19]\n\t"
+        "v_mad_u64_u32 v[18:19], vcc, %[q3], s21, v[18:19]\n\t"
+        "v_mad_u64_u32 v[18:19], vcc, %[q4], s20, v[18:19]\n\t"
+        "v_mad_u64_u32 v[18:19], vcc, %[q5], s19, v[18:19]\n\t"
+        "v_mad_u64_u32 v[18:19], vcc, %[q6], s18, v[18:19]\n\t"
+        "v_mad_u64_u32 v[18:19], vcc, %[q7], s17, v[18:19]\n\t"
+        "v_mad_u64_u32 v[18:19], vcc, %[q8], s16, v[18:19]\n\t"
+        "v_and_b32 %[r8], s26, v18\n\t"
+        : [r0] "+v"(r[0]), [r1] "+v"(r[1]), [r2] "+v"(r[2]), [r3] "+v"(r[3]), [r4] "+v"(r[4]), [r5] "+v"(r[5]), [r6] "+v"(r[6]), [r7] "+v"(r[7]), [r8] "+v"(r[8]), [q0] "=&v"(q[0]), [q1] "=&v"(q[1]), [q2] "=&v"(q[2]), [q3] "=&v"(q[3]), [q4] "=&v"(q[4]), [q5] "=&v"(q[5]), [q6] "=&v"(q[6]), [q7] "=&v"(q[7]), [q8] "=&v"(q[8])
+        : [v0] "v"(v[0]), [v1] "v"(v[1]), [v2] "v"(v[2]), [v3] "v"(v[3]), [v4] "v"(v[4]), [v5] "v"(v[5]), [v6] "v"(v[6]), [v7] "v"(v[7]), [v8] "v"(v[8]), [w0] "v"(w[0]), [w1] "v"(w[1]), [w2] "v"(w[2]), [w3] "v"(w[3]), [w4] "v"(w[4]), [w5] "v"(w[5]), [w6] "v"(w[6]), [w7] "v"(w[7]), [w8] "v"(w[8])
+        : "v16", "v17", "v18", "v19", "s16", "s17", "s18", "s19", "s20", "s21", "s22", "s23", "s24", "s25", "s26", "vcc");
 }
+}
diff --git a/ezkl_amd/csrc/ntt.hip b/ezkl_amd/csrc/ntt.hip
--- a/ezkl_amd/csrc/ntt.hip
+++ b/ezkl_amd/csrc/ntt.hip
@@ -23,8 +23,8 @@
     fe_t zeta[2];
     fe_t post_c[3];
     uint32_t cm, cm_log_e, cm_first, cm_log_cnt;
-    const f29_t* tw_stage29;
-    const f29_t* tw_pre29;
+    const tw29_t* tw_stage29;
+    const tw29_t* tw_pre29;
     uint32_t lds_stages;
 };
 
@@ -45,7 +45,7 @@
     return x;
 }
 template <int G, int NTT_THREADS, bool FROM_TABLE>
-__device__ __forceinline__ void ntt_superstage29(uint2* data, uint32_t* d8, const f29_t* tw, uint32_t TILE, uint32_t logC, bool unit1, uint32_t s, uint32_t tid) {
+__device__ __forceinline__ void ntt_superstage29(uint2* data, uint32_t* d8, const tw29_t* tw, uint32_t TILE, uint32_t logC, bool unit1, uint32_t s, uint32_t tid) {
     constexpr uint32_t M = 1u << G;
     const uint32_t C = 1u << logC;
     const uint32_t lh = s - 1, h = 1u << lh;
@@ -74,8 +74,8 @@
                     x[i] = Fr29::add(x[i], v);
                 } else {
                     const uint32_t off = o + (i & (half - 1)) * h;
-                    const f29_t w = ld_f29(tw + base + off);
-                    const f29_t v = Fr29::mul(x[i + half], w);
+                    const tw29_t* e = tw + base + off;
+                    const f29_t v = Fr29::mulc(x[i + half], ld_f29(&e->w), ld_f29(&e->q));
                     x[i + half] = Fr29::sub<1>(x[i], v);
                     x[i] = Fr29::add(x[i], v);
                 }
@@ -94,7 +94,7 @@
     const uint32_t log_s = a.log_m - a.log_r, S = 1u << log_s;
     uint2* data = reinterpret_cast<uint2*>(smem);
     uint32_t* d8 = reinterpret_cast<uint32_t*>(smem + 32u * TILE);
-    f29_t* tloc = reinterpret_cast<f29_t*>(smem + 36u * TILE);
+    tw29_t* tloc = reinterpret_cast<tw29_t*>(smem + 36u * TILE);
     const uint32_t tid = threadIdx.x, tile = blockIdx.x;
     const uint32_t cm_l = a.cm ? (blockIdx.y & ((1u << a.cm_log_cnt) - 1u)) : 0u, cm_col = a.cm ? (blockIdx.y >> a.cm_log_cnt) : blockIdx.y;
     const uint32_t cm_b = a.cm_first + cm_l;
@@ -102,8 +102,11 @@
     const fe_t* in = a.in + (size_t)(twisted ? cm_col : blockIdx.y) * a.in_stride;
     fe_t* out = (a.cm && a.last) ? a.out + (size_t)cm_col * a.out_stride + ((size_t)cm_l << a.log_n) : a.out + (size_t)blockIdx.y * a.out_stride;
     const fe_t* tw_inter = a.tw_inter ? a.tw_inter + (twisted ? ((size_t)cm_b << a.log_n) : 0) : nullptr;
-    const f29_t* tws = twisted ? a.tw_pre29 + ((size_t)cm_b << a.log_r) : a.tw_stage29;
-    for (uint32_t j = tid; j + 1 < (1u << a.lds_stages); j += NTT_THREADS) st_f29(tloc + j, ld_f29(tws + j));
+    const tw29_t* tws = twisted ? a.tw_pre29 + ((size_t)cm_b << a.log_r) : a.tw_stage29;
+    for (uint32_t j = tid; j + 1 < (1u << a.lds_stages); j += NTT_THREADS) {
+        st_f29(&tloc[j].w, ld_f29(&tws[j].w));
+        st_f29(&tloc[j].q, ld_f29(&tws[j].q));
+    }
 
     uint32_t n_blocks = 1u << (a.log_n - a.log_r);
     uint32_t sblk = a.npass >= 2 ? (n_blocks >> a.log_radix[0]) : 1u;
@@ -221,7 +224,7 @@
 }
 
 
-__global__ void ntt_coset_table_kernel(fe_t* out, f29_t* out29, uint32_t cnt, uint32_t log_e, uint32_t log_ext, uint32_t log_s, int mode, const fe_t* pow2tab,
+__global__ void ntt_coset_table_kernel(fe_t* out, tw29_t* out29, uint32_t cnt, uint32_t log_e, uint32_t log_ext, uint32_t log_s, int mode, const fe_t* pow2tab,
                                        fe_t z0, fe_t z1, fe_t z2) {
     const size_t idx = (size_t)blockIdx.x * blockDim.x + threadIdx.x;
     if (idx >= ((size_t)cnt << log_e)) return;
@@ -232,8 +235,10 @@
         while (((uint64_t)1 << st) - 1 <= m) st++;
         const uint64_t o = m - (((uint64_t)1 << (st - 1)) - 1), log_nn = log_ext - log_e;
         if (st > log_nn) {
-            if (out29) st_f29(out29 + idx, Fr29::zero());
-            else st_fe(out + idx, Fr::zero());
+            if (out29) {
+                st_f29(&out29[idx].w, Fr29::zero());
+                st_f29(&out29[idx].q, Fr29::zero());
+            } else st_fe(out + idx, Fr::zero());
             return;
         }
         const uint64_t q = (uint64_t)1 << (log_nn - st);
@@ -248,8 +253,12 @@
     fe_t acc = z == 0 ? z0 : (z == 1 ? z1 : z2);
     for (uint32_t q = 0; q < log_ext; q++)
         if ((e >> q) & 1) acc = Fr::mul(acc, ld_fe(pow2tab + q));
-    if (out29) st_f29(out29 + idx, Fr29::unpack(acc));
-    else st_fe(out + idx, acc);
+    if (out29) {
+        f29_t w, wq;
+        Fr29::mulc_pair(Fr29::unpack(acc), w, wq);
+        st_f29(&out29[idx].w, w);
+        st_f29(&out29[idx].q, wq);
+    } else st_fe(out + idx, acc);
 }
 __global__ __launch_bounds__(256) void ntt_cm_transpose_kernel(const fe_t* in, fe_t* out, uint32_t log_n, uint32_t log_e, int to_natural) {
     const size_t j = (size_t)blockIdx.x * blockDim.x + threadIdx.x;
@@ -267,12 +276,12 @@
     int npass = 0;
     uint32_t log_radix[4] = {0, 0, 0, 0};
     fe_t* tw_inter[4] = {nullptr, nullptr, nullptr, nullptr};
-    f29_t* stage29 = nullptr;
+    tw29_t* stage29 = nullptr;
     fe_t n_inv;
 };
 
 struct CosetTables {
-    f29_t* pre29 = nullptr;
+    tw29_t* pre29 = nullptr;
     fe_t* inter = nullptr;
 };
 struct NttState {
@@ -288,8 +297,8 @@
 #define g_plans (ntt_state().plans)
 #define g_coset_tables (ntt_state().coset_tables)
 
-static uint32_t ntt_lds_stages(uint32_t log_r) { return log_r < 6 ? log_r : 6; }
-static size_t ntt_lds_bytes(uint32_t log_tile, uint32_t log_r) { return 36u * ((size_t)1 << log_tile) + 36u * ((size_t)1 << ntt_lds_stages(log_r)); }
+static uint32_t ntt_lds_stages(uint32_t log_r) { return log_r < 4 ? log_r : 4; }
+static size_t ntt_lds_bytes(uint32_t log_tile, uint32_t log_r) { return 36u * ((size_t)1 << log_tile) + sizeof(tw29_t) * ((size_t)1 << ntt_lds_stages(log_r)); }
 static fe_t ntt_domain_one() { return Fr::from_u64(32); }
 
 static uint32_t ntt_max_radix() {
@@ -352,7 +361,7 @@
         uint32_t maxlr = 0;
         for (int i = 0; i < p->npass; i++) maxlr = p->log_radix[i] > maxlr ? p->log_radix[i] : maxlr;
         const uint32_t cnt = 1u << maxlr;
-        EZ_HIP(hipMalloc(&p->stage29, sizeof(f29_t) * cnt));
+        EZ_HIP(hipMalloc(&p->stage29, sizeof(tw29_t) * cnt));
         hipLaunchKernelGGL(ntt_coset_table_kernel, dim3(cdiv(cnt, 256)), dim3(256), 0, st, (fe_t*)nullptr, p->stage29, cnt, 0u, log_n, 0u, 0, d_pow2, one, one, one);
     }
     for (int i = 0; i < p->npass; i++) {
@@ -475,18 +484,39 @@
     CosetTables t;
     const fe_t one = ntt_domain_one(), zeta = Fr::mul(fr_const(FrConst::ZETA), one), zeta2 = Fr::mul(fr_const(FrConst::ZETA2), one);
     const size_t n_pre = (size_t)1 << (lr + log_e);
-    EZ_HIP(hipMalloc(&t.pre29, sizeof(f29_t) * n_pre));
+    EZ_HIP(hipMalloc(&t.pre29, sizeof(tw29_t) * n_pre));
     hipLaunchKernelGGL(ntt_coset_table_kernel, dim3(cdiv(n_pre, 256)), dim3(256), 0, st, (fe_t*)nullptr, t.pre29, 1u << lr, log_e, log_ext, log_s, 0, d_pow2, one, zeta, zeta2);
     if (p->npass > 1) {
         const size_t n_int = (size_t)1 << log_ext;
         EZ_HIP(hipMalloc(&t.inter, sizeof(fe_t) * n_int));
-        hipLaunchKernelGGL(ntt_coset_table_kernel, dim3(cdiv(n_int, 256)), dim3(256), 0, st, t.inter, (f29_t*)nullptr, 1u << log_n, log_e, log_ext, log_s, 1, d_pow2, one, zeta, zeta2);
+        hipLaunchKernelGGL(ntt_coset_table_kernel, dim3(cdiv(n_int, 256)), dim3(256), 0, st, t.inter, (tw29_t*)nullptr, 1u << log_n, log_e, log_ext, log_s, 1, d_pow2, one, zeta, zeta2);
     }
     EZ_HIP(hipGetLastError());
     EZ_HIP(hipStreamSynchronize(st));
     EZ_HIP(hipFree(d_pow2));
     g_coset_tables[key] = t;
     *out = t;
+    return EZKL_OK;
+}
+
+int ntt_tables_download(Ctx* c, hipStream_t st, uint32_t log_n, uint32_t log_ext, const fe_t& w_n, const fe_t& w_ext, void* out, size_t capacity, size_t* count) {
+    NttPlan* p = nullptr;
+    int rc = plan_get(c, st, log_n, w_n, &p);
+    if (rc) return rc;
+    const tw29_t* src = p->stage29;
+    uint32_t maxlr = 0;
+    for (int i = 0; i < p->npass; i++) maxlr = p->log_radix[i] > maxlr ? p->log_radix[i] : maxlr;
+    size_t n = (size_t)1 << maxlr;
+    if (log_ext) {
+        CosetTables ct;
+        if ((rc = coset_tables_get(c, st, p, log_n, log_ext, w_ext, &ct))) return rc;
+        src = ct.pre29;
+        n = (size_t)1 << (p->log_radix[0] + log_ext - log_n);
+    }
+    *count = n;
+    if (capacity < n) return EZKL_ERR_INVALID;
+    EZ_HIP(hipMemcpyAsync(out, src, n * sizeof(tw29_t), hipMemcpyDeviceToHost, st));
+    EZ_HIP(hipStreamSynchronize(st));
     return EZKL_OK;
 }
 
diff --git a/ezkl_amd/csrc/ubench.hip b/ezkl_amd/csrc/ubench.hip
--- a/ezkl_amd/csrc/ubench.hip
+++ b/ezkl_amd/csrc/ubench.hip
@@ -201,6 +201,38 @@
     }
     uint32_t x = 0;
     for (int i = 0; i < 9; i++) x ^= a[i] ^ b[i] ^ c[i] ^ d[i];
+    io[t * 8] = x;
+}
+__global__ __launch_bounds__(256) void ub_mulc29_kernel(uint32_t* io, int iters, uint32_t* mismatches) {
+    size_t t = (size_t)blockIdx.x * blockDim.x + threadIdx.x;
+    f29_t a, c, W1, W2;
+    for (int i = 0; i < 9; i++) {
+        uint32_t x = io[t * 8 + (i & 7)] * 2654435761u + i + (uint32_t)t * 40503u;
+        a.v[i] = x & 0x1fffffffu; W1.v[i] = (x >> 3) & 0x1fffffffu; c.v[i] = (x * 7u) & 0x1fffffffu; W2.v[i] = (x * 13u) & 0x1fffffffu;
+    }
+    a.v[8] &= 0x3fffu; W1.v[8] &= 0x3fffu; c.v[8] &= 0x3fffu; W2.v[8] &= 0x3fffu;
+    f29_t w1, q1, w2, q2;
+    Fr29::mulc_pair(W1, w1, q1);
+    Fr29::mulc_pair(W2, w2, q2);
+    if (mismatches) {
+        bool bad = false;
+        f29_t loose = Fr29::add(Fr29::add(a, a), Fr29::add(c, c));
+        const f29_t got[3] = {Fr29::mulc(a, w1, q1), Fr29::mulc(c, w2, q2), Fr29::mulc(loose, w1, q1)};
+        const f29_t want[3] = {Fr29::mul(a, W1), Fr29::mul(c, W2), Fr29::mul(loose, W1)};
+        for (int j = 0; j < 3; j++) {
+            const f29_t g = Fr29::canonical(got[j]), w = Fr29::canonical(want[j]);
+            for (int i = 0; i < 9; i++) bad |= g.v[i] != w.v[i];
+        }
+        if (bad) atomicAdd(mismatches, 1u);
+    }
+    for (int k = 0; k < iters; k++) {
+        a = Fr29::mulc(a, w1, q1);
+        c = Fr29::mulc(c, w2, q2);
+        a = Fr29::mulc(a, w2, q2);
+        c = Fr29::mulc(c, w1, q1);
+    }
+    uint32_t x = 0;
+    for (int i = 0; i < 9; i++) x ^= a.v[i] ^ c.v[i];
     io[t * 8] = x;
 }
 
@@ -548,7 +580,7 @@
         *out = chk ? (double)hm : 4.0 * iters * (double)nthreads / (ms * 1e-3);
         return EZKL_OK;
     }
-    if (!strncmp(which, "modmul29", 8)) {
+    if (!strncmp(which, "modmul29", 8) || !strncmp(which, "mulc29", 6)) {
         void* buf = nullptr;
         uint32_t* mis = nullptr;
         EZ_HIP(hipMalloc(&buf, nthreads * 32));
@@ -562,7 +594,8 @@
         const size_t nthreads = (size_t)blocks * threads;
         for (int rep = 0; rep < 2; rep++) {
             EZ_HIP(hipEventRecord(e0, st));
-            if (!strncmp(which, "modmul29i", 9)) hipLaunchKernelGGL(ub_modmul29i_kernel, dim3(blocks), dim3(threads), 0, st, (uint32_t*)buf, iters, chk ? mis : nullptr);
+            if (!strncmp(which, "mulc29", 6)) hipLaunchKernelGGL(ub_mulc29_kernel, dim3(blocks), dim3(threads), 0, st, (uint32_t*)buf, iters, chk ? mis : nullptr);
+            else if (!strncmp(which, "modmul29i", 9)) hipLaunchKernelGGL(ub_modmul29i_kernel, dim3(blocks), dim3(threads), 0, st, (uint32_t*)buf, iters, chk ? mis : nullptr);
             else hipLaunchKernelGGL(ub_modmul29_kernel, dim3(blocks), dim3(threads), 0, st, (uint32_t*)buf, iters, chk ? mis : nullptr);
             EZ_HIP(hipEventRecord(e1, st));
             EZ_HIP(hipStreamSynchronize(st));
diff --git a/ezkl_amd/lib.py b/ezkl_amd/lib.py
--- a/ezkl_amd/lib.py
+++ b/ezkl_amd/lib.py
@@ -10,7 +10,7 @@
     "ezkl_hip_memcpy_d2h", "ezkl_hip_bases_upload", "ezkl_hip_bases_prepare", "ezkl_hip_bases_free", "ezkl_hip_bases_len", "ezkl_hip_bases_generate",
     "ezkl_hip_bases_download", "ezkl_hip_bases_from_scalars", "ezkl_hip_bases_downsize", "ezkl_hip_msm_g2", "ezkl_hip_msm_g1",
     "ezkl_hip_msm_g1_dev", "ezkl_hip_msm_g1_start_dev", "ezkl_hip_msm_g1_finish", "ezkl_hip_msm_g1_batch", "ezkl_hip_msm_g1_batch_dev", "ezkl_hip_msm_g1_batch_small_dev", "ezkl_hip_g1_add_affine", "ezkl_hip_ntt", "ezkl_hip_ntt_dev",
-    "ezkl_hip_coset_ntt_batch", "ezkl_hip_coset_ntt_dev", "ezkl_hip_coeff_to_cosets_dev", "ezkl_hip_coeff_to_cosets_range_dev", "ezkl_hip_cosets_transpose_dev", "ezkl_hip_vec_op_dev", "ezkl_hip_vec_scale_dev", "ezkl_hip_permutation_sigma_dev", "ezkl_hip_vec_fill_dev", "ezkl_hip_host_malloc", "ezkl_hip_host_free", "ezkl_hip_upload_commit_batch", "ezkl_hip_upload_begin", "ezkl_hip_upload_begin_fmt", "ezkl_hip_upload_wait", "ezkl_hip_upload_commit", "ezkl_hip_upload_end", "ezkl_hip_msm_batch_begin", "ezkl_hip_msm_batch_push_dev", "ezkl_hip_msm_batch_push_many_dev", "ezkl_hip_msm_batch_finish", "ezkl_hip_eval_poly_batch_dev", "ezkl_hip_lincomb_dev", "ezkl_hip_kate_division_dev", "ezkl_hip_chacha20_fr_dev",
+    "ezkl_hip_coset_ntt_batch", "ezkl_hip_coset_ntt_dev", "ezkl_hip_coeff_to_cosets_dev", "ezkl_hip_coeff_to_cosets_range_dev", "ezkl_hip_cosets_transpose_dev", "ezkl_hip_ntt_tables_download", "ezkl_hip_vec_op_dev", "ezkl_hip_vec_scale_dev", "ezkl_hip_permutation_sigma_dev", "ezkl_hip_vec_fill_dev", "ezkl_hip_host_malloc", "ezkl_hip_host_free", "ezkl_hip_upload_commit_batch", "ezkl_hip_upload_begin", "ezkl_hip_upload_begin_fmt", "ezkl_hip_upload_wait", "ezkl_hip_upload_commit", "ezkl_hip_upload_end", "ezkl_hip_msm_batch_begin", "ezkl_hip_msm_batch_push_dev", "ezkl_hip_msm_batch_push_many_dev", "ezkl_hip_msm_batch_finish", "ezkl_hip_eval_poly_batch_dev", "ezkl_hip_lincomb_dev", "ezkl_hip_kate_division_dev", "ezkl_hip_chacha20_fr_dev",
     "ezkl_hip_divide_by_vanishing_dev", "ezkl_hip_prefix_scan_dev", "ezkl_hip_eval_poly_dev", "ezkl_hip_lookup_multiplicity_dev", "ezkl_hip_lookup_multiplicity_acc_dev", "ezkl_hip_lookup_multiplicity_batch_dev", "ezkl_hip_batch_invert_dev", "ezkl_hip_eval_h_dev", "ezkl_hip_eval_h_check", "ezkl_hip_eval_h_source", "ezkl_hip_eval_h_schedule", "ezkl_hip_eval_h_prepare", "ezkl_hip_eval_h_jit_stats", "ezkl_hip_eval_check_dev", "ezkl_hip_eval_check_source", "ezkl_hip_lookup_missing_rows_dev", "ezkl_hip_copy_check_dev", "ezkl_hip_set_async", "ezkl_hip_stream_wait_library",
     "ezkl_hip_last_kernel_ms", "ezkl_hip_kernel_ms_stats", "ezkl_hip_ubench",
     "ezkl_hip_witness_plan_upload", "ezkl_hip_witness_plan_free", "ezkl_hip_witness_plan_info", "ezkl_hip_witness_run_dev", "ezkl_hip_witness_last_error",
diff --git a/include/ezkl_hip.h b/include/ezkl_hip.h
--- a/include/ezkl_hip.h
+++ b/include/ezkl_hip.h
@@ -108,6 +108,7 @@
 int ezkl_hip_coeff_to_cosets_dev(const void* in_dev, void* out_dev, size_t batch, size_t in_stride_elems, size_t out_stride_elems,
                                  uint32_t log_n, uint32_t log_n_ext, void* stream);
 int ezkl_hip_cosets_transpose_dev(const void* in_dev, void* out_dev, uint32_t log_n, uint32_t log_n_ext, int to_natural, void* stream);
+int ezkl_hip_ntt_tables_download(uint32_t log_n, uint32_t log_n_ext, void* out_host, size_t capacity_entries, size_t* count);
 int ezkl_hip_coeff_to_cosets_range_dev(const void* in_dev, void* out_dev, size_t batch, size_t in_stride_elems, size_t out_stride_elems,
                                        uint32_t log_n, uint32_t log_n_ext, uint32_t first_coset, uint32_t n_cosets, void* stream);
 
```
